# genjax-dev/genjax-chi

Measured on AMD Instinct MI355X. Metric: particles/sec, ImportanceK log-marginal-likelihood estimate (1e6 particles per GPU), higher is better.
Workload: dtype f32

## Files before the change

### genjax-chi_amd/csrc/gjx_device.hpp

```cpp
#pragma once
#ifndef __HIPCC_RTC__
#include <hip/hip_runtime.h>
#include <stdint.h>
#else
typedef unsigned char uint8_t;
typedef unsigned short uint16_t;
typedef int int32_t;
typedef unsigned int uint32_t;
typedef long long int64_t;
typedef unsigned long long uint64_t;
typedef unsigned long uintptr_t;
typedef unsigned long size_t;
#endif

#define GJX_DEV __device__ __forceinline__
#define GJX_HD __host__ __device__ __forceinline__

namespace gjx {

constexpr int kWave = 64;
constexpr int kBlock = 256;
#ifndef GJX_TILE
#define GJX_TILE 1024
#endif
// ... 237 lines not shown
  if (s.mode == 2) return s.parent;
  return split_at<IMPL>(s.parent, s.first + i);
}
template <int IMPL>
GJX_DEV void store_key(uint32_t* out, uint64_t i, Key k) {
  if (IMPL == 0) reinterpret_cast<uint2*>(out)[i] = make_uint2(k.k0, k.k1);
  else reinterpret_cast<uint4*>(out)[i] = make_uint4(k.k0, k.k1, k.l0, k.l1);
}

#if defined(__HIP_DEVICE_COMPILE__)
GJX_DEV float opq(float x) {
  asm volatile("" : "+v"(x));
  return x;
}
#else
GJX_HD float opq(float x) { return x; }
#endif

GJX_HD float m_log(float x) {
  uint32_t ix = f2u(x);
  int32_t e = 0;
  if (ix - 1u >= 0x7f7fffffu) {
    if ((ix << 1) == 0u) return -__builtin_inff();
    return ix == 0x7f800000u ? x : u2f(0x7fc00000u);
  }
  if (ix < 0x00800000u) {
    x = x * 8388608.0f;
    ix = f2u(x);
    e = -23;
  }
  const uint32_t t = ix - 0x3f3504f3u;
  e += (int32_t)t >> 23;
  const float m = u2f((t & 0x007fffffu) + 0x3f3504f3u);
  const float f = m - 1.0f;
  const float z = f * f;
  float p = 7.0376836292E-2f;
  p = __builtin_fmaf(p, f, -1.1514610310E-1f);
  p = __builtin_fmaf(p, f, 1.1676998740E-1f);
  p = __builtin_fmaf(p, f, -1.2420140846E-1f);
  p = __builtin_fmaf(p, f, 1.4249322787E-1f);
  p = __builtin_fmaf(p, f, -1.6668057665E-1f);
  p = __builtin_fmaf(p, f, 2.0000714765E-1f);
  p = __builtin_fmaf(p, f, -2.4999993993E-1f);
  p = __builtin_fmaf(p, f, 3.3333331174E-1f);
  float y = (p * f) * z;
  const float fe = (float)e;
  y = __builtin_fmaf(fe, -2.12194440e-4f, y);
  y = __builtin_fmaf(-0.5f, z, y);
  float r = f + y;
  r = __builtin_fmaf(fe, 0.693359375f, r);
  return r;
}

GJX_HD float m_log_normal(float x) {
  const uint32_t t = f2u(x) - 0x3f3504f3u;
  const int32_t e = (int32_t)t >> 23;
  const float m = u2f((t & 0x007fffffu) + 0x3f3504f3u);
  const float f = m - 1.0f;
  const float z = f * f;
  float p = 7.0376836292E-2f;
  p = __builtin_fmaf(p, f, -1.1514610310E-1f);
  p = __builtin_fmaf(p, f, 1.1676998740E-1f);
  p = __builtin_fmaf(p, f, -1.2420140846E-1f);
  p = __builtin_fmaf(p, f, 1.4249322787E-1f);
  p = __builtin_fmaf(p, f, -1.6668057665E-1f);
  p = __builtin_fmaf(p, f, 2.0000714765E-1f);
  p = __builtin_fmaf(p, f, -2.4999993993E-1f);
  p = __builtin_fmaf(p, f, 3.3333331174E-1f);
  float y = (p * f) * z;
  const float fe = (float)e;
  y = __builtin_fmaf(fe, -2.12194440e-4f, y);
  y = __builtin_fmaf(-0.5f, z, y);
  float r = f + y;
  r = __builtin_fmaf(fe, 0.693359375f, r);
  return r;
}

GJX_HD float m_exp_core(float x);
GJX_HD float m_exp(float x) {
  if (!(x >= -86.0f)) return 0.0f;
  if (x > 88.0f) x = 88.0f;
  return m_exp_core(x);
}
GJX_HD float m_exp_core(float x) {
  const float fx = __builtin_rintf(x * 1.44269504088896341f);
  x = __builtin_fmaf(fx, -0.693359375f, x);
  x = __builtin_fmaf(fx, 2.12194440e-4f, x);
  const float z = x * x;
  float p = 1.9875691500E-4f;
  p = __builtin_fmaf(p, x, 1.3981999507E-3f);
  p = __builtin_fmaf(p, x, 8.3334519073E-3f);
  p = __builtin_fmaf(p, x, 4.1665795894E-2f);
  p = __builtin_fmaf(p, x, 1.6666665459E-1f);
  p = __builtin_fmaf(p, x, 5.0000001201E-1f);
  const float y = __builtin_fmaf(p, z, x) + 1.0f;
  const int32_t n = (int32_t)fx;
  return u2f(f2u(y) + ((uint32_t)n << 23));
}

GJX_HD float e_exp(float x) {
  if (x != x) return x;
  if (x > 88.0f || x < -86.0f) {
    const float h = m_exp(x * 0.5f);
    return h * h;
  }
  return m_exp(x);
}

GJX_HD float e_max(float a, float b) { return (a != a) ? a : ((b != b) ? b : (a > b ? a : b)); }
GJX_HD float e_min(float a, float b) { return (a != a) ? a : ((b != b) ? b : (a < b ? a : b)); }

#if defined(GJX_FAST_MATH) && defined(__HIP_DEVICE_COMPILE__)
#define GJX_FAST_MATH_DEVICE 1
GJX_HD float d_exp(float x) { return __builtin_amdgcn_exp2f(x * 1.44269504088896341f); }
GJX_HD float d_exp_core(float x) { return d_exp(x); }
#else
GJX_HD float d_exp(float x) { return m_exp(x); }
GJX_HD float d_exp_core(float x) { return m_exp_core(x); }
#endif

GJX_HD float m_erfinv(float x) {
  float w = -m_log_normal((1.0f - x) * (1.0f + x));
  float p;
  if (w < 5.0f) {
    w = w - 2.5f;
    p = 2.81022636e-08f;
    p = __builtin_fmaf(p, w, 3.43273939e-07f);
    p = __builtin_fmaf(p, w, -3.5233877e-06f);
    p = __builtin_fmaf(p, w, -4.39150654e-06f);
    p = __builtin_fmaf(p, w, 0.00021858087f);
    p = __builtin_fmaf(p, w, -0.00125372503f);
    p = __builtin_fmaf(p, w, -0.00417768164f);
    p = __builtin_fmaf(p, w, 0.246640727f);
    p = __builtin_fmaf(p, w, 1.50140941f);
  } else {
    w = __builtin_sqrtf(w) - 3.0f;
    p = -0.000200214257f;
    p = __builtin_fmaf(p, w, 0.000100950558f);
    p = __builtin_fmaf(p, w, 0.00134934322f);
    p = __builtin_fmaf(p, w, -0.00367342844f);
    p = __builtin_fmaf(p, w, 0.00573950773f);
    p = __builtin_fmaf(p, w, -0.0076224613f);
    p = __builtin_fmaf(p, w, 0.00943887047f);
    p = __builtin_fmaf(p, w, 1.00167406f);
    p = __builtin_fmaf(p, w, 2.83297682f);
  }
  return p * x;
}

GJX_HD float m_lgamma(float x) {
  float p = 1.0f;
#pragma unroll
  for (int i = 0; i < 8; ++i) {
    if (x < 8.0f) {
      p = p * x;
      x = x + 1.0f;
    }
  }
  const float xi = 1.0f / x;
  const float xi2 = xi * xi;
  float s = __builtin_fmaf(xi2, 7.9365079365e-4f, -2.7777777778e-3f);
  s = __builtin_fmaf(s, xi2, 8.3333333333e-2f);
  s = s * xi;
  float r = (x - 0.5f) * m_log(x);
  r = r - x;
  r = r + 0.91893853320467f;
  r = r + s;
  r = r - m_log(p);
  return r;
}

GJX_HD float uniform01(uint32_t bits) { return u2f((bits >> 9) | 0x3F800000u) - 1.0f; }

GJX_HD float std_normal(uint32_t bits) {
  const float lo = -0.99999994f;
  float u = uniform01(bits) * 2.0f + lo;
  u = u > lo ? u : lo;
  return 1.41421356237309505f * m_erfinv(u);
}

struct BmEnt {
// ... 57 lines not shown
  {0xbf6b4b0cu, 0xbec9b953u}, {0xbf68bf3cu, 0xbed53641u}, {0xbf660f88u, 0xbee0924fu}, {0xbf633c5au, 0xbeebcbbbu}, \
  {0xbf604621u, 0xbef6e0cbu}, {0xbf5d2d53u, 0xbf00e7e4u}, {0xbf59f26au, 0xbf064b82u}, {0xbf5695e5u, 0xbf0b9a6bu}, \
  {0xbf531849u, 0xbf10d3cdu}, {0xbf4f7a1fu, 0xbf15f6d9u}, {0xbf4bbbf8u, 0xbf1b02c6u}, {0xbf47de65u, 0xbf1ff6cbu}, \
  {0xbf43e200u, 0xbf24d225u}, {0xbf3fc767u, 0xbf299415u}, {0xbf3b8f3bu, 0xbf2e3bdeu}, {0xbf373a23u, 0xbf32c8c9u}, \
  {0xbf32c8c9u, 0xbf373a23u}, {0xbf2e3bdeu, 0xbf3b8f3bu}, {0xbf299415u, 0xbf3fc767u}, {0xbf24d225u, 0xbf43e200u}, \
  {0xbf1ff6cbu, 0xbf47de65u}, {0xbf1b02c6u, 0xbf4bbbf8u}, {0xbf15f6d9u, 0xbf4f7a1fu}, {0xbf10d3cdu, 0xbf531849u}, \
  {0xbf0b9a6bu, 0xbf5695e5u}, {0xbf064b82u, 0xbf59f26au}, {0xbf00e7e4u, 0xbf5d2d53u}, {0xbef6e0cbu, 0xbf604621u}, \
  {0xbeebcbbbu, 0xbf633c5au}, {0xbee0924fu, 0xbf660f88u}, {0xbed53641u, 0xbf68bf3cu}, {0xbec9b953u, 0xbf6b4b0cu}, \
  {0xbebe1d4au, 0xbf6db293u}, {0xbeb263efu, 0xbf6ff573u}, {0xbea68f12u, 0xbf721352u}, {0xbe9aa086u, 0xbf740bddu}, \
  {0xbe8e9a22u, 0xbf75dec6u}, {0xbe827dc0u, 0xbf778bc5u}, {0xbe6c9a7fu, 0xbf791298u}, {0xbe541501u, 0xbf7a7302u}, \
  {0xbe3b6ecfu, 0xbf7baccdu}, {0xbe22abb6u, 0xbf7cbfc9u}, {0xbe09cf86u, 0xbf7dabccu}, {0xbde1bc2eu, 0xbf7e70b0u}, \
  {0xbdafb680u, 0xbf7f0e58u}, {0xbd7b2b74u, 0xbf7f84abu}, {0xbd16c32cu, 0xbf7fd397u}, {0xbc490e90u, 0xbf7ffb11u}, \
  {0x3c490e90u, 0xbf7ffb11u}, {0x3d16c32cu, 0xbf7fd397u}, {0x3d7b2b74u, 0xbf7f84abu}, {0x3dafb680u, 0xbf7f0e58u}, \
  {0x3de1bc2eu, 0xbf7e70b0u}, {0x3e09cf86u, 0xbf7dabccu}, {0x3e22abb6u, 0xbf7cbfc9u}, {0x3e3b6ecfu, 0xbf7baccdu}, \
  {0x3e541501u, 0xbf7a7302u}, {0x3e6c9a7fu, 0xbf791298u}, {0x3e827dc0u, 0xbf778bc5u}, {0x3e8e9a22u, 0xbf75dec6u}, \
  {0x3e9aa086u, 0xbf740bddu}, {0x3ea68f12u, 0xbf721352u}, {0x3eb263efu, 0xbf6ff573u}, {0x3ebe1d4au, 0xbf6db293u}, \
  {0x3ec9b953u, 0xbf6b4b0cu}, {0x3ed53641u, 0xbf68bf3cu}, {0x3ee0924fu, 0xbf660f88u}, {0x3eebcbbbu, 0xbf633c5au}, \
  {0x3ef6e0cbu, 0xbf604621u}, {0x3f00e7e4u, 0xbf5d2d53u}, {0x3f064b82u, 0xbf59f26au}, {0x3f0b9a6bu, 0xbf5695e5u}, \
  {0x3f10d3cdu, 0xbf531849u}, {0x3f15f6d9u, 0xbf4f7a1fu}, {0x3f1b02c6u, 0xbf4bbbf8u}, {0x3f1ff6cbu, 0xbf47de65u}, \
  {0x3f24d225u, 0xbf43e200u}, {0x3f299415u, 0xbf3fc767u}, {0x3f2e3bdeu, 0xbf3b8f3bu}, {0x3f32c8c9u, 0xbf373a23u}, \
  {0x3f373a23u, 0xbf32c8c9u}, {0x3f3b8f3bu, 0xbf2e3bdeu}, {0x3f3fc767u, 0xbf299415u}, {0x3f43e200u, 0xbf24d225u}, \
  {0x3f47de65u, 0xbf1ff6cbu}, {0x3f4bbbf8u, 0xbf1b02c6u}, {0x3f4f7a1fu, 0xbf15f6d9u}, {0x3f531849u, 0xbf10d3cdu}, \
  {0x3f5695e5u, 0xbf0b9a6bu}, {0x3f59f26au, 0xbf064b82u}, {0x3f5d2d53u, 0xbf00e7e4u}, {0x3f604621u, 0xbef6e0cbu}, \
  {0x3f633c5au, 0xbeebcbbbu}, {0x3f660f88u, 0xbee0924fu}, {0x3f68bf3cu, 0xbed53641u}, {0x3f6b4b0cu, 0xbec9b953u}, \
  {0x3f6db293u, 0xbebe1d4au}, {0x3f6ff573u, 0xbeb263efu}, {0x3f721352u, 0xbea68f12u}, {0x3f740bddu, 0xbe9aa086u}, \
  {0x3f75dec6u, 0xbe8e9a22u}, {0x3f778bc5u, 0xbe827dc0u}, {0x3f791298u, 0xbe6c9a7fu}, {0x3f7a7302u, 0xbe541501u}, \
  {0x3f7baccdu, 0xbe3b6ecfu}, {0x3f7cbfc9u, 0xbe22abb6u}, {0x3f7dabccu, 0xbe09cf86u}, {0x3f7e70b0u, 0xbde1bc2eu}, \
  {0x3f7f0e58u, 0xbdafb680u}, {0x3f7f84abu, 0xbd7b2b74u}, {0x3f7fd397u, 0xbd16c32cu}, {0x3f7ffb11u, 0xbc490e90u}, \
}
#if defined(__HIP_DEVICE_COMPILE__)
static __device__ const BmEnt g_bm_lg[64] = GJX_BM_LG_INIT;
static __device__ const BmEnt g_bm_cs[256] = GJX_BM_CS_INIT;
#else
static const BmEnt g_bm_lg[64] = GJX_BM_LG_INIT;
static const BmEnt g_bm_cs[256] = GJX_BM_CS_INIT;
#endif
#if defined(GJX_BM_LDS) && defined(__HIP_DEVICE_COMPILE__)
__shared__ BmEnt s_bm_lg[64];
__shared__ BmEnt s_bm_cs[256];
#ifndef GJX_BM_BLOCK
#error "GJX_BM_LDS needs GJX_BM_BLOCK: the size of the workgroups that call bm_stage()"
#endif
struct BmLoads {
  BmEnt c[256 / GJX_BM_BLOCK], l;
  GJX_DEV void bm_stage() const {
    constexpr int BD = GJX_BM_BLOCK, K = 256 / BD;
    const uint32_t t = threadIdx.x;
#pragma unroll
    for (int k = 0; k < K; ++k) s_bm_cs[t + (uint32_t)(k * BD)] = c[k];
    if (BD == 64 || t < 64u) s_bm_lg[t] = l;
    __syncthreads();
  }
};
GJX_DEV BmLoads bm_issue() {
  constexpr int BD = GJX_BM_BLOCK, K = 256 / BD;
  static_assert(BD == 64 || BD == 128 || BD == 256, "workgroups have 64, 128 or 256 threads");
  const uint32_t t = threadIdx.x;
  BmLoads r;
  r.l = BmEnt{0u, 0u};
#pragma unroll
  for (int k = 0; k < K; ++k) r.c[k] = g_bm_cs[t + (uint32_t)(k * BD)];
  if (BD == 64 || t < 64u) r.l = g_bm_lg[t];
  return r;
}
GJX_DEV void bm_stage() { bm_issue().bm_stage(); }
#define GJX_BM_LG s_bm_lg
#define GJX_BM_CS s_bm_cs
#else
#define GJX_BM_LG g_bm_lg
#define GJX_BM_CS g_bm_cs
#endif
GJX_HD float sqrt_pos(float x) {
#if defined(__HIP_DEVICE_COMPILE__) && !defined(GJX_GENERAL_SQRT)
  const float y = __builtin_amdgcn_rsqf(__builtin_fmaxf(x, 1e-30f));
  float s = x * y, h = 0.5f * y;
  const float e = __builtin_fmaf(-h, s, 0.5f);
  h = __builtin_fmaf(h, e, h);
  s = __builtin_fmaf(s, e, s);
  return __builtin_fmaf(__builtin_fmaf(-s, s, x), h, s);
#else
  return __builtin_sqrtf(x);
#endif
}
GJX_HD void bm_pair(uint32_t w_radius, uint32_t w_angle, float& z_cos, float& z_sin) {
  const float uw = (float)w_radius + 1.0f;
#ifdef GJX_FAST_MATH_DEVICE
  {
    const float u = uw * 2.3283064365386963e-10f;
    const float rf = __builtin_amdgcn_sqrtf(-1.38629436111989062f * __builtin_amdgcn_logf(u));
    const float tf = (float)(w_angle >> 8) * 5.9604644775390625e-08f;
    z_cos = rf * __builtin_amdgcn_cosf(tf);
    z_sin = rf * __builtin_amdgcn_sinf(tf);
    return;
  }
#endif
  const uint32_t t = f2u(uw) - (0x3f3504f3u + (32u << 23));
  const BmEnt lg = GJX_BM_LG[(t >> 17) & 63u];
  const float m = u2f((t & 0x007fffffu) + 0x3f3504f3u);
  const float fe = (float)((int32_t)t >> 23);
  const float q = __builtin_fmaf(m, u2f(lg.a), -1.0f);
  float p = __builtin_fmaf(q, -0.25f, 0.333333343f);
  p = __builtin_fmaf(p, q, -0.5f);
  const float l1 = __builtin_fmaf(p, q * q, q);
  const float lu = __builtin_fmaf(fe, 0.693147182f, u2f(lg.b)) + l1;
  const float r = sqrt_pos(-2.0f * lu);
  const BmEnt cs = GJX_BM_CS[w_angle >> 24];
  const float d = __builtin_fmaf((float)((w_angle >> 8) & 0xffffu), 3.74507035e-07f, -0.0122718466f);
  const float d2 = d * d;
  const float sd = __builtin_fmaf(d2 * d, -0.166666672f, d);
  const float cd = __builtin_fmaf(d2, __builtin_fmaf(d2, 0.0416666679f, -0.5f), 1.0f);
  const float ca = u2f(cs.a), sa = u2f(cs.b);
  z_cos = r * __builtin_fmaf(ca, cd, -(sa * sd));
  z_sin = r * __builtin_fmaf(sa, cd, ca * sd);
}
constexpr uint32_t kTagTwin = 0x54u;
template <int IMPL>
GJX_HD float site_normal(const Stream<IMPL>& st) {
  if (IMPL == 0 || !st.hf) return std_normal(st.bits32(0));
  float zc, zs;
  uint32_t o[4];
  if ((st.k.l0 | st.k.l1) == 0u) {
    philox4x32(st.k.k0, st.k.k1, 0u, 0u, st.f >> 2, kTagTwin, o[0], o[1], o[2], o[3]);
    const uint32_t sel = st.f & 3u;
    bm_pair(philox_single_draw(st.k, st.f), sel == 0 ? o[0] : (sel == 1 ? o[1] : (sel == 2 ? o[2] : o[3])), zc, zs);
    return zc;
  }
  philox_pair_block(st.k, st.f >> 1, o);
  if (st.f & 1u) bm_pair(o[2], o[3], zc, zs);
  else bm_pair(o[0], o[1], zc, zs);
  return ((st.k.l0 - 1u) & 1u) ? zs : zc;
}

template <int IMPL>
GJX_HD void smc_quad_normals(Key step_key, uint64_t g, float (&z)[4]) {
  uint32_t w[4];
  smc_quad_bits<IMPL>(step_key, g, w);
  if (IMPL == 0) {
#pragma unroll
    for (int u = 0; u < 4; ++u) z[u] = std_normal(w[u]);
  } else {
    bm_pair(w[0], w[1], z[0], z[1]);
    bm_pair(w[2], w[3], z[2], z[3]);
  }
}
template <int IMPL>
GJX_HD float smc_slot_normal(Key step_key, uint64_t j) {
  if (IMPL == 0) return std_normal(smc_slot_bits<IMPL>(step_key, j));
  float z[4];
  smc_quad_normals<IMPL>(step_key, j >> 2, z);
  const uint32_t sel = (uint32_t)j & 3u;
  return sel == 0 ? z[0] : (sel == 1 ? z[1] : (sel == 2 ? z[2] : z[3]));
}

GJX_HD float normal_rs(float scale) { return 1.0f / scale; }
GJX_HD float normal_lognorm(float scale) { return 0.91893853320467f + m_log(scale); }
GJX_HD float logpdf_normal_pre(float x, float loc, float rs, float lognorm) {
  const float d = x * rs - loc * rs;
  return (-0.5f * d) * d - lognorm;
}
GJX_HD float logpdf_normal(float x, float loc, float scale) {
  return logpdf_normal_pre(x, loc, normal_rs(scale), normal_lognorm(scale));
}
GJX_HD float normal_resid_pow2(float x, float loc, float rs) { return __builtin_fmaf(-rs, loc, x * rs); }
GJX_HD float normal_halfsq(float d, float lognorm) { return __builtin_fmaf(d * d, -0.5f, -lognorm); }
struct NormalExactCuts {};
GJX_HD float logpdf_normal_pre(float x, float loc, float rs, float lognorm, NormalExactCuts) {
  return normal_halfsq(normal_resid_pow2(x, loc, rs), lognorm);
}
GJX_HD float xlogy(float a, float y) { return a == 0.0f ? 0.0f : a * m_log(y); }
GJX_HD float gamma_lognorm(float conc, float rate) { return m_lgamma(conc) - conc * m_log(rate); }
GJX_HD float logpdf_gamma_pre(float x, float conc, float rate, float lognorm) {
  return (xlogy(conc - 1.0f, x) - rate * x) - lognorm;
}
GJX_HD float logpdf_gamma(float x, float conc, float rate) {
  return logpdf_gamma_pre(x, conc, rate, gamma_lognorm(conc, rate));
}
GJX_HD float beta_lbeta(float a, float b) { return (m_lgamma(a) + m_lgamma(b)) - m_lgamma(a + b); }
GJX_HD float logpdf_beta_pre(float x, float a, float b, float lbeta) {
  return (xlogy(a - 1.0f, x) + xlogy(b - 1.0f, 1.0f - x)) - lbeta;
}
GJX_HD float logpdf_beta(float x, float a, float b) {
  return logpdf_beta_pre(x, a, b, beta_lbeta(a, b));
}
GJX_HD float logpdf_bernoulli(bool e, float p) { return e ? m_log(p) : m_log(1.0f - p); }

template <int IMPL>
GJX_DEV float gamma_dv(const Stream<IMPL>& st, int which, float conc) {
  const bool boost = conc < 1.0f;
  const float a = boost ? conc + 1.0f : conc;
  const float d = a - 0.33333334f;
  const float c = 1.0f / __builtin_sqrtf(9.0f * d);
  float v = 1.0f;
  for (int att = 0; att < 64; ++att) {
    uint32_t w0, w1;
    st.words((uint32_t)(1 + 2 * att + which), w0, w1);
    const float x = std_normal(w0);
// ... 59 lines not shown
  v = (t * t) * t;
  const float u = uniform01(w1);
  float rhs = (0.5f * x) * x + d;
  rhs = rhs - d * v;
  rhs = rhs + d * m_log(v);
  return m_log(u) < rhs;
}
template <int IMPL, int P>
GJX_DEV void std_gamma_multi(const Stream<IMPL> (&st)[P], int which, const float (&conc)[P], float (&out)[P]) {
  float d[P], c[P], v[P];
  int att[P];
  bool done[P];
#pragma unroll
  for (int u = 0; u < P; ++u) {
    const float a = conc[u] < 1.0f ? conc[u] + 1.0f : conc[u];
    d[u] = a - 0.33333334f;
    c[u] = 1.0f / __builtin_sqrtf(9.0f * d[u]);
    v[u] = 1.0f;
  }
#pragma unroll
  for (int u = 0; u < P; ++u) {
    done[u] = gamma_attempt<IMPL>(st[u], which, 0, d[u], c[u], v[u]);
    att[u] = 1;
  }
  for (;;) {
    int pick = -1;
#pragma unroll
    for (int u = P - 1; u >= 0; --u) pick = (!done[u] && att[u] < 64) ? u : pick;
#if defined(__HIP_DEVICE_COMPILE__)
    if (__ballot(pick >= 0) == 0) break;
#else
    if (pick < 0) break;
#endif
    if (pick >= 0) {
      Stream<IMPL> s = st[0];
      float dd = d[0], cc = c[0], vv = v[0];
      int aa = att[0];
#pragma unroll
      for (int u = 1; u < P; ++u)
        if (pick == u) { s = st[u]; dd = d[u]; cc = c[u]; vv = v[u]; aa = att[u]; }
      const bool ok = gamma_attempt<IMPL>(s, which, aa, dd, cc, vv);
#pragma unroll
      for (int u = 0; u < P; ++u)
        if (pick == u) { v[u] = vv; att[u] = aa + 1; done[u] = ok; }
    }
  }
#pragma unroll
  for (int u = 0; u < P; ++u) {
    float g = d[u] * v[u];
    if (conc[u] < 1.0f) {
      uint32_t w0, w1;
      st[u].words(0u, w0, w1);
      const float ub = uniform01(which ? w1 : w0);
      g = g * m_exp(m_log(ub) / conc[u]);
    }
    out[u] = g;
  }
}

GJX_HD uint64_t fixw(float lw, float m, int frac) {
  if (lw == m) return (uint64_t)1 << frac;
  const float d = lw - m;
  if (!(d >= -80.0f)) return 0;
  const float s = m_exp(d);
  const float t = s * u2f((uint32_t)(127 + frac) << 23);
  return (uint64_t)__builtin_rintf(t);
}
constexpr int kRowFrac = 30;
constexpr int32_t kRowEmpty = -(1 << 30);
constexpr int kLseBuckets = 64;
constexpr int kLseRecordWords = 1 + kLseBuckets;
GJX_HD int32_t row_anchor(float m) {
  if (!(m > -__builtin_inff())) return kRowEmpty;
  float t = m * 1.44269504088896341f;
  t = t > 16777216.0f ? 16777216.0f : (t < -16777216.0f ? -16777216.0f : t);
  return (int32_t)__builtin_ceilf(t);
}
GJX_HD uint64_t rowfix(float lw, int32_t e) {
#if defined(__HIP_DEVICE_COMPILE__)
  {
    const float fe = (float)e;
    float d = __builtin_fmaf(-fe, 0.693359375f, lw);
    d = __builtin_fmaf(-fe, -2.12194440e-4f, d);
    d = d > 1.0f ? 1.0f : d;
    const bool live = e != kRowEmpty && lw > -__builtin_inff() && d >= -86.0f;
    const uint32_t q = (uint32_t)__builtin_rintf(d_exp_core(live ? d : 0.0f) * 1073741824.0f);
    return live ? q : 0u;
  }
#endif
  if (e == kRowEmpty || !(lw > -__builtin_inff())) return 0;
  const float fe = (float)e;
  float d = __builtin_fmaf(-fe, 0.693359375f, lw);
  d = __builtin_fmaf(-fe, -2.12194440e-4f, d);
  d = d > 1.0f ? 1.0f : d;
  return (uint64_t)(uint32_t)__builtin_rintf(d_exp(d) * 1073741824.0f);
}

GJX_HD uint32_t cat_fix(float l, float m) {
  if (l == m) return 1u << kCatFrac;
  const float d = l - m;
  if (!(d >= -80.0f)) return 0u;
  return (uint32_t)__builtin_rintf(m_exp(d) * 8388608.0f);
}
GJX_HD int frac_bits(uint64_t n_total) {
  int lg = 0;
  while (lg < 63 && ((uint64_t)1 << lg) < n_total) ++lg;
  const int f = 62 - lg;
  return f > 40 ? 40 : (f < 8 ? 8 : f);
}
GJX_HD float gumbel_from_bits(uint32_t bits) {
  const float tiny = 1.17549435e-38f;
  float u = uniform01(bits) + tiny;
  u = u > tiny ? u : tiny;
  return -m_log(-m_log(u));
}

#if defined(__HIP_DEVICE_COMPILE__)
GJX_DEV float jrow_max(const float* l, uint32_t K) {
  float m = l[0];
  for (uint32_t c = 1; c < K; ++c) m = l[c] > m ? l[c] : m;
  return m;
}
GJX_DEV float jrow_lse(const float* l, uint32_t K) {
  const float m = jrow_max(l, K);
  float acc = 0.0f;
  for (uint32_t c = 0; c < K; ++c) acc = acc + m_exp(l[c] - m);
  return m + m_log(acc);
}
GJX_DEV int32_t jcat_invcdf(const float* l, uint32_t K, uint32_t bits) {
  const float m = jrow_max(l, K);
  uint64_t Q = 0;
  for (uint32_t c = 0; c < K; ++c) Q += cat_fix(l[c], m);
  const uint64_t thr = (uint64_t)bits * (Q >> 32) + (((uint64_t)bits * (Q & 0xffffffffu)) >> 32);
  uint64_t C = 0;
  for (uint32_t c = 0; c < K; ++c) {
    C += cat_fix(l[c], m);
    if (C > thr) return (int32_t)c;
  }
  return (int32_t)(K - 1);
}
typedef unsigned jv4u_t __attribute__((ext_vector_type(4)));
GJX_DEV uint4 jguide_load(const uint4* p) {
  const uint64_t a = (uint64_t)(uintptr_t)p;
  const uint64_t first = ((uint64_t)(uint32_t)__builtin_amdgcn_readfirstlane((int)(uint32_t)(a >> 32)) << 32) |
                         (uint64_t)(uint32_t)__builtin_amdgcn_readfirstlane((int)(uint32_t)a);
  const uint64_t base = first - (1ull << 30);
  __amdgpu_buffer_rsrc_t rs = __builtin_amdgcn_make_buffer_rsrc((void*)(uintptr_t)base, 0, 0x7fffffff, 0x00020000);
  const jv4u_t v = __builtin_amdgcn_raw_buffer_load_b128(rs, (int)(uint32_t)(a - base), 0, 0);
  return make_uint4(v[0], v[1], v[2], v[3]);
}
GJX_DEV int32_t jcat_invcdf_gb(const uint4* guide, const uint2* ent, uint32_t K, uint32_t bits, int sh, uint32_t& lpb) {
  const uint4 g = jguide_load(guide + (bits >> sh));
  const uint32_t c0 = g.y & 511u, c1 = (g.y >> 9) & 511u;
  if (bits <= g.x) {
    lpb = g.z;
    return (int32_t)c0;
  }
  if (!(g.y >> 18)) {
    lpb = g.w;
    return (int32_t)c1;
  }
  const uint64_t thr = ((uint64_t)bits * (uint64_t)ent[K - 1].x) >> 32;
  uint32_t c = c1;
  uint2 e = ent[c];
  while (c < K - 1 && (uint64_t)e.x <= thr) {
    ++c;
    e = ent[c];
  }
  lpb = e.y;
  return (int32_t)c;
}
template <int IMPL>
GJX_DEV int32_t jcat_gumbel(const float* l, uint32_t K, const Stream<IMPL>& st) {
  int32_t best = 0;
  float bv = -__builtin_inff();
  for (uint32_t c = 0; c < K; ++c) {
    const float v = l[c] + gumbel_from_bits(st.bits32(c));
    if (v > bv || c == 0) {
      bv = v;
      best = (int32_t)c;
    }
  }
  return best;
}
#endif

GJX_HD int64_t teeth_below(uint64_t C, double scale, double u0, int64_t n_out) {
  const double P = (double)C * scale;
  const double c = __builtin_ceil(P - u0);
  if (!(c > 0.0)) return 0;
  if (c >= (double)n_out) return n_out;
  return (int64_t)(int32_t)c;
}
GJX_HD double u0_from_bits(uint64_t U) { return (double)(U >> 11) * 0x1.0p-53; }

template <int CTRL, int ROW_MASK, int BANK_MASK>
GJX_DEV uint32_t dpp_u32(uint32_t identity, uint32_t v) {
  return (uint32_t)__builtin_amdgcn_update_dpp((int)identity, (int)v, CTRL, ROW_MASK, BANK_MASK, false);
}
template <int CTRL, int ROW_MASK, int BANK_MASK>
GJX_DEV uint64_t dpp_u64(uint64_t identity, uint64_t v) {
  const uint32_t lo = dpp_u32<CTRL, ROW_MASK, BANK_MASK>((uint32_t)identity, (uint32_t)v);
  const uint32_t hi = dpp_u32<CTRL, ROW_MASK, BANK_MASK>((uint32_t)(identity >> 32), (uint32_t)(v >> 32));
  return ((uint64_t)hi << 32) | lo;
}
constexpr int kDppRowShr1 = 0x111, kDppRowShr2 = 0x112, kDppRowShr3 = 0x113, kDppRowShr4 = 0x114, kDppRowShr8 = 0x118,
              kDppRowBcast15 = 0x142, kDppRowBcast31 = 0x143, kDppWaveShr1 = 0x138;
#define GJX_WAVE_SCAN_BODY(T, MOV)                                               \
  T r = op(v, MOV<kDppRowShr1, 0xf, 0xf>(id, v));                                \
  r = op(r, MOV<kDppRowShr2, 0xf, 0xf>(id, v));                                  \
  r = op(r, MOV<kDppRowShr3, 0xf, 0xf>(id, v));                                  \
  r = op(r, MOV<kDppRowShr4, 0xf, 0xe>(id, r));                                  \
  r = op(r, MOV<kDppRowShr8, 0xf, 0xc>(id, r));                                  \
  r = op(r, MOV<kDppRowBcast15, 0xa, 0xf>(id, r));                               \
  r = op(r, MOV<kDppRowBcast31, 0xc, 0xf>(id, r));                               \
  return r;
template <class Op>
GJX_DEV uint32_t wave_scan_u32(uint32_t v, uint32_t id, Op op) { GJX_WAVE_SCAN_BODY(uint32_t, dpp_u32) }
template <class Op>
GJX_DEV uint64_t wave_scan_u64(uint64_t v, uint64_t id, Op op) { GJX_WAVE_SCAN_BODY(uint64_t, dpp_u64) }
#undef GJX_WAVE_SCAN_BODY
GJX_DEV uint32_t wave_last_u32(uint32_t v) { return (uint32_t)__builtin_amdgcn_readlane((int)v, 63); }
GJX_DEV uint64_t wave_last_u64(uint64_t v) {
  return ((uint64_t)wave_last_u32((uint32_t)(v >> 32)) << 32) | wave_last_u32((uint32_t)v);
}
GJX_DEV float wave_max(float v) {
  v = v == v ? v : -__builtin_inff();
  const uint32_t r = wave_scan_u32(f2u(v), f2u(-__builtin_inff()),
                                   [](uint32_t a, uint32_t b) { return u2f(b) > u2f(a) ? b : a; });
  return u2f(wave_last_u32(r));
}
GJX_DEV uint64_t wave_sum(uint64_t v) {
  return wave_last_u64(wave_scan_u64(v, 0, [](uint64_t a, uint64_t b) { return a + b; }));
}
GJX_DEV int wave_sum_int(int v) {
  return (int)wave_last_u32(wave_scan_u32((uint32_t)v, 0u, [](uint32_t a, uint32_t b) { return a + b; }));
}
GJX_DEV float block_max(float v, float* sh) {
  v = wave_max(v);
  const int w = threadIdx.x >> 6;
  __syncthreads();
  if ((threadIdx.x & 63) == 0) sh[w] = v;
  __syncthreads();
  float r = sh[0];
#pragma unroll
  for (int i = 1; i < kBlock / kWave; ++i) r = sh[i] > r ? sh[i] : r;
  return r;
}
GJX_DEV uint64_t block_sum(uint64_t v, uint64_t* sh) {
  v = wave_sum(v);
  const int w = threadIdx.x >> 6;
  __syncthreads();
  if ((threadIdx.x & 63) == 0) sh[w] = v;
  __syncthreads();
  uint64_t r = 0;
#pragma unroll
  for (int i = 0; i < kBlock / kWave; ++i) r += sh[i];
  return r;
}
GJX_DEV uint64_t wave_scan_incl(uint64_t v) {
  return wave_scan_u64(v, 0, [](uint64_t a, uint64_t b) { return a + b; });
}
GJX_DEV uint64_t wave_scan_incl_52(uint64_t v) {
  const uint32_t lo = wave_scan_u32((uint32_t)v & 0x3ffffffu, 0u, [](uint32_t a, uint32_t b) { return a + b; });
  const uint32_t hi = wave_scan_u32((uint32_t)(v >> 26), 0u, [](uint32_t a, uint32_t b) { return a + b; });
  return ((uint64_t)hi << 26) + lo;
}
GJX_DEV uint64_t wave_sum_52(uint64_t v) { return wave_last_u64(wave_scan_incl_52(v)); }
GJX_DEV uint64_t block_scan_excl(uint64_t v, uint64_t* sh, uint64_t& total) {
  const uint64_t incl = wave_scan_incl(v);
  const int w = threadIdx.x >> 6, lane = threadIdx.x & 63;
  __syncthreads();
  if (lane == 63) sh[w] = incl;
  __syncthreads();
  uint64_t base = 0, tot = 0;
#pragma unroll
  for (int i = 0; i < kBlock / kWave; ++i) {
    if (i < w) base += sh[i];
    tot += sh[i];
  }
  total = tot;
  return base + incl - v;
}

GJX_DEV int block_scan_max_excl(int v, int* sh) {
  const int lane = threadIdx.x & 63, w = threadIdx.x >> 6;
  const int incl = (int)wave_scan_u32((uint32_t)v, 0u, [](uint32_t a, uint32_t b) { return b > a ? b : a; });
  int excl = (int)dpp_u32<kDppWaveShr1, 0xf, 0xf>(0u, (uint32_t)incl);
  __syncthreads();
  if (lane == 63) sh[w] = incl;
  __syncthreads();
#pragma unroll
  for (int i = 0; i < kBlock / kWave; ++i)
    if (i < w) excl = sh[i] > excl ? sh[i] : excl;
  return excl;
}
GJX_DEV int block_sum_int(int v, int* sh) {
  v = wave_sum_int(v);
  __syncthreads();
  if ((threadIdx.x & 63) == 0) sh[threadIdx.x >> 6] = v;
  __syncthreads();
  int r = 0;
#pragma unroll
  for (int i = 0; i < kBlock / kWave; ++i) r += sh[i];
  return r;
}

constexpr int kMaxFilters = 16;
struct FilterBatch {
  uint32_t n_filters = 0;
  uint32_t tiles = 0;
  uint64_t stride = 0;
  uint64_t mq_stride = 0;
// ... 1421 lines not shown
```

### genjax-chi_amd/csrc/gjx_hip.hip

```cpp
#include "../../include/gjx.h"
#include "../../include/gjx_guided.h"
#include "../../include/gjx_backsim.h"
#include "../../include/gjx_backmove.h"
#include "../../include/gjx_smc_params.h"
#include "../../include/gjx_csmc.h"
#include "../../include/gjx_temper.h"
#include "../../include/gjx_plate.h"
#include "../../include/gjx_pointwise.h"
#include "../../include/gjx_temper_cov.h"
#define GJX_PHILOX_PLAIN_XOR 1
#include "gjx_device.hpp"

#include <hip/hip_runtime.h>
#include <math.h>
#include <new>
#include <string.h>

#include "gjx_plan_jit.hpp"

using namespace gjx;

namespace {

inline int launch_status() { return hipGetLastError() == hipSuccess ? GJX_OK : GJX_ERR_LAUNCH; }
// ... 1581 lines not shown
    scaled[c] = p * (uint64_t)K;
    alias[c] = (uint16_t)c;
    q += p;
  }
  q = wave_sum(q);
  if ((tid & 63) == 0) sh_q[tid >> 6] = q;
  __syncthreads();
  const uint64_t Q = sh_q[0] + sh_q[1];
  if (tid == 0) {
    uint32_t hs = 0, ts = 0, hl = 0, tl = 0;
    for (int c = 0; c < K; ++c) {
      if (scaled[c] < Q) small[ts++] = (uint16_t)c;
      else large[tl++] = (uint16_t)c;
    }
    while (hs < ts && hl < tl) {
      const uint32_t sc = small[hs++], g = large[hl];
      alias[sc] = (uint16_t)g;
      scaled[g] -= Q - scaled[sc];
      if (scaled[g] < Q) {
        ++hl;
        small[ts++] = (uint16_t)g;
      }
    }
  } else if (tid == 64) {
    const float* o = obs_logits + (size_t)r * K;
    sh_lse = row_lse(o, (uint32_t)K);
  }
  __syncthreads();
  uint32_t* row = trans_alias + (size_t)r * K;
  for (int c = tid; c < K; c += 128) {
    const uint32_t thr = alias[c] == c ? 0xffffffu : (uint32_t)((scaled[c] << 24) / Q);
    row[c] = (thr << 8) | alias[c];
    obs_logp[(size_t)r * K + c] = obs_logits[(size_t)r * K + c] - sh_lse;
  }
}

struct Carver {
  char* p;
  size_t left;
  bool ok = true;
  template <class T>
  T* take(size_t count) {
    const size_t bytes = (count * sizeof(T) + 255) & ~(size_t)255;
    if (!ok || bytes > left) {
      ok = false;
      return nullptr;
    }
    T* r = reinterpret_cast<T*>(p);
    p += bytes;
    left -= bytes;
    return r;
  }
};
inline size_t pad256(size_t b) { return (b + 255) & ~(size_t)255; }

template <int OP>
__global__ __launch_bounds__(kBlock) void k_map_f32(const float* x, float c, float* out, uint64_t n) {
  const uint64_t i0 = ((uint64_t)blockIdx.x * kBlock + threadIdx.x) * 4;
#pragma unroll
  for (int r = 0; r < 4; ++r) {
    const uint64_t i = i0 + r;
    if (i < n) {
      const float v = x[i];
      out[i] = OP == GJX_MAP_EXP ? e_exp(v) : OP == GJX_MAP_LOG ? m_log(v) : OP == GJX_MAP_DIV ? v / c : OP == GJX_MAP_RDIV ? c / v
               : OP == GJX_MAP_SQRT ? __builtin_sqrtf(v) : __builtin_fabsf(v);
    }
  }
}

__global__ __launch_bounds__(kBlock) void k_sqrt_pos_sweep(uint32_t lo, uint64_t count, unsigned long long* out) {
  unsigned long long bad = 0, first = ~0ull;
  for (uint64_t i = (uint64_t)blockIdx.x * kBlock + threadIdx.x; i < count; i += (uint64_t)gridDim.x * kBlock) {
    const uint32_t b = lo + (uint32_t)i;
    if (f2u(sqrt_pos(u2f(b))) != f2u(__builtin_sqrtf(u2f(b)))) {
      ++bad;
      first = first < b ? first : b;
    }
  }
  if (bad) {
    atomicAdd(&out[0], bad);
    atomicMin(&out[1], first);
  }
}
}

static int copy_source_out(const std::string& src, char* buf, size_t buf_len, size_t* needed) {
  if (needed) *needed = src.size() + 1;
  if (buf && buf_len > 0) {
    const size_t k = src.size() < buf_len - 1 ? src.size() : buf_len - 1;
    memcpy(buf, src.data(), k);
    buf[k] = 0;
  }
  return GJX_OK;
}
static int version_out(int* major, int* minor, int maj, int min) {
  if (major) *major = maj;
  if (minor) *minor = min;
  return GJX_OK;
}
extern "C" {

int gjx_version(int* major, int* minor) { return version_out(major, minor, GJX_VERSION_MAJOR, GJX_VERSION_MINOR); }
const char* gjx_backend_name(void) { return "hip-gfx950"; }
int gjx_frac_bits(uint64_t n_total) { return frac_bits(n_total); }
uint64_t gjx_smc_tile(void) { return kTile; }
uint64_t gjx_num_tiles(uint64_t n) { return ntiles_of(n); }
uint64_t gjx_num_max_partials(uint64_t n) { return nrows_of(n); }

size_t gjx_workspace_bytes(int op, uint64_t n) {
  const uint64_t nt = ntiles_of(n);
  switch (op) {
    case GJX_OP_LOGSUMEXP: return pad256(nrows_of(n) * 4) + pad256(nt * 8) + 1024;
    case GJX_OP_CATEGORICAL_INDEX:
    case GJX_OP_RESAMPLE:
      return pad256(nt * 4) + 2 * pad256(nt * 8) + pad256(n * 8) + pad256(nt * 160) + pad256(prefix_words(nt) * 8) + 2048;
    case GJX_OP_SMC:
      return (GJX_SMC_MAX_STATE + 3) * pad256(n * 4) + 2 * (pad256(nt * 16) + pad256(nt * 128) + pad256(nt * 16)) + 2 * pad256(prefix_words(nt) * 8) + 4096 +
             pad256(256 * (256 + 64) * 4) + pad256(256 * 256 * 4) + 1024;
    default: return 0;
  }
}

#define GJX_DISPATCH_IMPL(impl, KERNEL, ...)  \
  do {                                        \
    if ((impl) == 0) KERNEL<0> __VA_ARGS__;   \
    else KERNEL<1> __VA_ARGS__;               \
  } while (0)

int gjx_rng_keys(const gjx_keys* k, uint64_t n, uint32_t* out, gjx_stream s) {
  if (!keys_ok(k) || (!out && n)) return GJX_ERR_INVALID;
  if (n == 0) return GJX_OK;
  GJX_DISPATCH_IMPL(k->impl, k_rng_keys, <<<grid_for(n), kBlock, 0, S(s)>>>(key_src(k), n, out));
  return launch_status();
}
int gjx_rng_split_each(const gjx_keys* k, uint64_t n, uint32_t m, uint32_t* out, gjx_stream s) {
  if (!keys_ok(k) || (!out && n) || m == 0) return GJX_ERR_INVALID;
  if (n == 0) return GJX_OK;
  GJX_DISPATCH_IMPL(k->impl, k_rng_split_each, <<<grid_for(n * m), kBlock, 0, S(s)>>>(key_src(k), n, m, out));
  return launch_status();
}
int gjx_rng_bits(const gjx_keys* k, uint32_t sub, uint64_t n, uint32_t* out, gjx_stream s) {
  if (!keys_ok(k) || (!out && n)) return GJX_ERR_INVALID;
  if (n == 0) return GJX_OK;
  GJX_DISPATCH_IMPL(k->impl, k_rng_bits, <<<grid_for(n), kBlock, 0, S(s)>>>(key_src(k), sub, n, out));
  return launch_status();
}

int gjx_sample_logpdf_normal(const gjx_keys* k, gjx_f32 loc, gjx_f32 scale, float* value_out,
                             float* score_out, uint64_t n, gjx_stream s) {
  if (!keys_ok(k) || !value_out) return GJX_ERR_INVALID;
  if (n == 0) return GJX_OK;
  GJX_DISPATCH_IMPL(k->impl, k_sample_normal,
                    <<<grid_for(n), kBlock, 0, S(s)>>>(key_src(k), opnd(loc), opnd(scale), value_out, score_out, n));
  return launch_status();
}
int gjx_sample_logpdf_gamma(const gjx_keys* k, gjx_f32 concentration, gjx_f32 rate,
                            float* value_out, float* score_out, uint64_t n, gjx_stream s) {
  if (!keys_ok(k) || !value_out) return GJX_ERR_INVALID;
  if (n == 0) return GJX_OK;
  GJX_DISPATCH_IMPL(k->impl, k_sample_gamma,
                    <<<grid_for(n), kBlock, 0, S(s)>>>(key_src(k), opnd(concentration), opnd(rate), value_out, score_out, n));
  return launch_status();
}
int gjx_sample_logpdf_beta(const gjx_keys* k, gjx_f32 a, gjx_f32 b, float* value_out,
                           float* score_out, uint64_t n, gjx_stream s) {
  if (!keys_ok(k) || !value_out) return GJX_ERR_INVALID;
// ... 84 lines not shown
    for (uint32_t k = c + 1; k < K; ++k)
      if (row[k].x > row[c].x) { cn = k; break; }
    const uint32_t last_bits = (uint32_t)((((uint64_t)g + 1) << sh) - 1);
    const uint64_t thr_last = ((uint64_t)last_bits * (uint64_t)C) >> 32;
    const bool multi = cn != c && (uint64_t)row[cn].x <= thr_last;
    const uint32_t bm1 = C == 0 ? 0xffffffffu : (uint32_t)(((((uint64_t)row[c].x) << 32) - 1) / (uint64_t)C);
    guide4[((size_t)r << gbits) + g] = make_uint4(row[c].x == 0 ? 0xffffffffu : bm1, c | (cn << 9) | ((multi ? 1u : 0u) << 18), row[c].y, row[cn].y);
  }
}
static void cat_tables_prepare(CSite* sites, int n, std::vector<void*>* owned) {
  bool any = false;
  for (int q = 0; q < n; ++q) {
    CSite& st = sites[q];
    if (st.dist != GJX_DIST_CATEGORICAL || st.cat_ent || st.cat_logp_t || !st.logits || st.n_cat > 511 || st.n_rows < 1) continue;
    const size_t rows = (size_t)st.n_rows;
    const unsigned grid = ((unsigned)rows + 63) / 64;
    if (!gjx_jit::sampled_mode(st.observed) && st.obs.kind != GJX_ARG_INPUT) {
      float* lt = nullptr;
      if (hipMalloc(&lt, sizeof(float) * rows * (size_t)st.n_cat) != hipSuccess) { (void)hipGetLastError(); continue; }
      k_cat_prepare<<<grid, 64>>>(st.logits, (uint32_t)rows, (uint32_t)st.n_cat, nullptr, nullptr, lt, 0);
      owned->push_back(lt);
      st.cat_logp_t = lt;
      any = true;
      continue;
    }
    uint2* ent = nullptr;
    uint4* guide4 = nullptr;
    int gbits = 8;
    while ((1 << gbits) < 4 * st.n_cat && gbits < 11) ++gbits;
    while (gbits > 8 && (sizeof(uint4) << gbits) * rows > ((size_t)2 << 20)) --gbits;
    if (hipMalloc(&ent, sizeof(uint2) * rows * (size_t)st.n_cat) != hipSuccess || hipMalloc(&guide4, (sizeof(uint4) << gbits) * rows) != hipSuccess) {
      (void)hipGetLastError();
      if (ent) (void)hipFree(ent);
      continue;
    }
    k_cat_prepare<<<grid, 64>>>(st.logits, (uint32_t)rows, (uint32_t)st.n_cat, ent, guide4, nullptr, gbits);
    owned->push_back(ent);
    owned->push_back(guide4);
    st.cat_ent = ent;
    st.cat_guide4 = guide4;
    st.cat_gbits = gbits;
    any = true;
  }
  if (any && hipDeviceSynchronize() != hipSuccess) (void)hipGetLastError();
}
static void free_owned(std::vector<void*>& owned) {
  for (void* p : owned) (void)hipFree(p);
  owned.clear();
}
struct SiteTable {
  CSite* sites;
  int n;
};
extern "C++" template <class Build>
static bool compiled_once(std::mutex& mu, gjx_jit::Module& c, std::initializer_list<SiteTable> tables, std::vector<void*>* owned,
                          Build build) {
  if (c.state == 0) {
    std::lock_guard<std::mutex> lock(mu);
    if (c.state == 0) {
      for (const SiteTable& t : tables) cat_tables_prepare(t.sites, t.n, owned);
      c.state = build() ? 1 : -1;
    }
  }
  return c.state == 1;
}

struct ExprStore {
  gjx_expr_op ops[GJX_MAX_SITES][2][GJX_MAX_EXPR_OPS];
};

struct gjx_plan {
  int n_sites;
  int n_slots;
  int dist_mask;
  uint32_t flags;
  int n_params;
  int max_param;
  PlanParams prm;
  CSite host[GJX_MAX_SITES];
  CSite* dev;
  gjx_jit::Compiled jit[4];
  gjx_jit::Compiled jit_tail[4];
  gjx_jit::Compiled jit_wt[2];
  std::vector<void*> dev_owned;
  std::mutex jit_mu;
  ExprStore expr;
  bool has_expr;
  int expr_max_input;
  gjx_jit::ScopeInfo scopes;
};

static bool expr_ok(const gjx_arg& a, int s, int n_state, int n_obs, bool allow_state, bool allow_param = false) {
  const gjx_expr_op* ops = reinterpret_cast<const gjx_expr_op*>(a.table);
  if (!ops || a.ref < 1 || a.ref > GJX_MAX_EXPR_OPS) return false;
  int depth = 0;
  for (int k = 0; k < a.ref; ++k) {
    const int r = ops[k].ref;
    switch (ops[k].op) {
      case GJX_EXPR_CONST: ++depth; break;
      case GJX_EXPR_SITE: if (r < 0 || r >= s) return false; ++depth; break;
      case GJX_EXPR_INPUT: if (n_state >= 0 || r < 0 || r >= 16) return false; ++depth; break;
      case GJX_EXPR_PARAM: if ((n_state >= 0 && !allow_param) || r < 0 || r >= GJX_MAX_PARAMS) return false; ++depth; break;
      case GJX_EXPR_STATE: if (n_state < 0 || !allow_state || r < 0 || r >= n_state) return false; ++depth; break;
      case GJX_EXPR_OBS: if (n_state < 0 || r < 0 || r >= n_obs) return false; ++depth; break;
      case GJX_EXPR_ADD: case GJX_EXPR_SUB: case GJX_EXPR_MUL: case GJX_EXPR_DIV: case GJX_EXPR_MAX: case GJX_EXPR_MIN:
      case GJX_EXPR_LT: case GJX_EXPR_LE: case GJX_EXPR_EQ:
        if (depth < 2) return false;
        --depth;
        break;
      case GJX_EXPR_SELECT:
        if (depth < 3) return false;
        depth -= 2;
        break;
      case GJX_EXPR_NEG: case GJX_EXPR_EXP: case GJX_EXPR_LOG: case GJX_EXPR_SQRT: case GJX_EXPR_ABS: if (depth < 1) return false; break;
      default: return false;
    }
    if (depth > 8) return false;
  }
  return depth == 1;
}

static bool arg_ok(const gjx_arg& a, int s, int n_state = -1, int n_obs = -1, bool allow_state = false, bool allow_param = false) {
  switch (a.kind) {
    case GJX_ARG_EXPR: return expr_ok(a, s, n_state, n_obs, allow_state, allow_param);
    case GJX_ARG_CONST: return true;
    case GJX_ARG_SITE: return a.ref >= 0 && a.ref < s;
    case GJX_ARG_INPUT: return n_state < 0 && a.ref >= 0 && a.ref < 16;
    case GJX_ARG_TABLE: return a.ref >= 0 && a.ref < s && a.table != nullptr;
    case GJX_ARG_STATE: return allow_state && a.ref >= 0 && a.ref < n_state;
    case GJX_ARG_OBS: return n_obs >= 0 && a.ref >= 0 && a.ref < n_obs;
    case GJX_ARG_PARAM: return (n_state < 0 || allow_param) && a.ref >= 0 && a.ref < GJX_MAX_PARAMS;
    default: return false;
  }
}
static CArg carg(const gjx_arg& a) { return CArg{a.kind, a.ref, 0, a.ref, a.scale, a.offset, a.table}; }

static bool convert_site(const gjx_site& st, int s, CSite& c, int n_state = -1, int n_obs = -1,
                         bool allow_state = false, bool allow_guided = false, bool allow_next = false, bool allow_param = false) {
  if (st.observed > (allow_guided ? GJX_SITE_GUIDED : 1)) return false;
  bool ok = st.dist >= 0 && st.dist <= GJX_DIST_CATEGORICAL && arg_ok(st.arg[0], s, n_state, n_obs, allow_state, allow_param);
  const bool two_args = st.dist != GJX_DIST_BERNOULLI && st.dist != GJX_DIST_CATEGORICAL;
  if (ok && two_args) ok = arg_ok(st.arg[1], s, n_state, n_obs, allow_state, allow_param);
  if (ok && st.observed == GJX_SITE_GUIDED) {
    ok = st.obs.kind == GJX_ARG_SITE && st.obs.ref >= 0 && st.obs.ref < s && st.obs.scale == 1.0f && st.obs.offset == 0.0f;
  } else if (ok && st.observed && st.observed != GJX_SITE_PROPOSED) {
    if (n_state < 0) ok = st.obs.kind == GJX_ARG_CONST || (st.obs.kind == GJX_ARG_INPUT && st.obs.ref >= 0 && st.obs.ref < 16) ||
                          (st.obs.kind == GJX_ARG_PARAM && st.obs.ref >= 0 && st.obs.ref < GJX_MAX_PARAMS);
    else ok = st.obs.kind == GJX_ARG_CONST || (st.obs.kind == GJX_ARG_OBS && st.obs.ref >= 0 && st.obs.ref < n_obs) ||
              (allow_param && st.obs.kind == GJX_ARG_PARAM && st.obs.ref >= 0 && st.obs.ref < GJX_MAX_PARAMS) ||
              (allow_next && st.obs.kind == GJX_ARG_NEXT && st.obs.ref >= 0 && st.obs.ref < n_state && st.obs.scale == 1.0f &&
               st.obs.offset == 0.0f);
  }
  if (ok && st.dist == GJX_DIST_CATEGORICAL)
    ok = st.logits && st.n_cat > 0 && st.n_rows > 0 && (st.cat_mode == 0 || st.cat_mode == 1) && st.arg[0].kind != GJX_ARG_EXPR;
  if (!ok) return false;
  memset(&c, 0, sizeof(c));
  c.dist = st.dist; c.observed = st.observed; c.out_col = st.out_col;
  c.n_cat = st.n_cat; c.n_rows = st.n_rows; c.cat_mode = st.cat_mode;
  c.slot = -1;
  c.a0 = carg(st.arg[0]); c.a1 = carg(st.arg[1]); c.obs = carg(st.obs);
  if (!two_args) c.a1.kind = GJX_ARG_CONST;
  c.logits = st.logits;
  const bool c0 = st.arg[0].kind == GJX_ARG_CONST, c1 = st.arg[1].kind == GJX_ARG_CONST;
  const bool u0 = c0 || st.arg[0].kind == GJX_ARG_PARAM, u1 = c1 || st.arg[1].kind == GJX_ARG_PARAM;
  if (st.dist == GJX_DIST_NORMAL && c1) {
    c.pre = 1; c.pre0 = normal_rs(st.arg[1].offset); c.pre1 = normal_lognorm(st.arg[1].offset);
// ... 81 lines not shown
        a->ref_is_int = p->host[a->ref].dist >= GJX_DIST_BERNOULLI;
        a->ref = site_slot[a->ref];
      }
    if (last_use[s] < 0) continue;
    int slot = -1;
    for (int k = 0; k < n_slots; ++k)
      if (slot_free_at[k] <= s) { slot = k; break; }
    if (slot < 0) slot = n_slots++;
    slot_free_at[slot] = last_use[s] + 1;
    site_slot[s] = slot;
    c.slot = slot;
  }
  p->n_slots = n_slots;
  p->has_expr = expr_adopt(p->host, n_sites, &p->expr);
  p->expr_max_input = expr_max_ref(p->host, n_sites, GJX_EXPR_INPUT);
  const int mp = expr_max_ref(p->host, n_sites, GJX_EXPR_PARAM);
  if (mp > p->max_param) p->max_param = mp;
  *out = p;
  return GJX_OK;
}

int gjx_plan_create_scoped(const gjx_site* sites, int n_sites, const gjx_scope* scopes, int n_scopes, uint32_t flags,
                           gjx_plan** out) {
  gjx_plan* p = nullptr;
  const int rc = gjx_plan_create_ex(sites, n_sites, flags, &p);
  if (rc) return rc;
  if (!gjx_jit::derive_scopes(sites, n_sites, scopes, n_scopes, p->scopes)) {
    gjx_plan_destroy(p);
    return GJX_ERR_INVALID;
  }
  *out = p;
  return GJX_OK;
}

static void plan_derive_params(PlanParams& prm, const CSite* sites, int n_sites) {
  auto val = [&](const CArg& a) {
    if (a.kind == GJX_ARG_CONST) return a.offset;
    const float t = a.scale * prm.p[a.ref];
    return t + a.offset;
  };
  for (int q = 0; q < n_sites; ++q) {
    const CSite& c = sites[q];
    if (c.pre != 2) continue;
    if (c.dist == GJX_DIST_NORMAL) {
      prm.d[2 * q] = normal_rs(val(c.a1));
      prm.d[2 * q + 1] = normal_lognorm(val(c.a1));
    } else if (c.dist == GJX_DIST_GAMMA) {
      prm.d[2 * q + 1] = gamma_lognorm(val(c.a0), val(c.a1));
    } else {
      prm.d[2 * q + 1] = beta_lbeta(val(c.a0), val(c.a1));
    }
  }
}
int gjx_plan_set_params(gjx_plan* p, const float* params, int n_params) {
  if (!p || n_params < 0 || n_params > GJX_MAX_PARAMS || (n_params && !params) || n_params <= p->max_param) return GJX_ERR_INVALID;
  for (int k = 0; k < n_params; ++k) p->prm.p[k] = params[k];
  p->n_params = n_params;
  plan_derive_params(p->prm, p->host, p->n_sites);
  return GJX_OK;
}

static int plan_device_table(gjx_plan* p) {
  std::lock_guard<std::mutex> lock(p->jit_mu);
  if (p->dev) return GJX_OK;
  if (hipMalloc(&p->dev, sizeof(CSite) * (size_t)p->n_sites) != hipSuccess) {
    p->dev = nullptr;
    return GJX_ERR_NO_DEVICE;
  }
  if (hipMemcpy(p->dev, p->host, sizeof(CSite) * (size_t)p->n_sites, hipMemcpyHostToDevice) != hipSuccess) {
    (void)hipFree(p->dev);
    p->dev = nullptr;
    return GJX_ERR_LAUNCH;
  }
  return GJX_OK;
}

static int jit_form_pref() {
  const char* e = std::getenv("GJX_JIT_FORM");
  if (e && !strcmp(e, "one")) return 1;
  if (e && !strcmp(e, "pair")) return 2;
  return 4;
}
static int jit_waves_hint(int P) { return P == 2 ? 6 : 0; }
static void plan_gen_setup(gjx_jit::Gen<CSite, CArg>& g, const gjx_plan* p, int impl, int form, bool fused_tail, bool wt_stores, int min_waves) {
  g.impl = impl; g.sites = p->host; g.n_sites = p->n_sites; g.laned = form >= 2; g.pairs_per_lane = form == 4 ? 2 : 1;
  g.sc = p->scopes.n_scopes > 0 ? &p->scopes : nullptr;
  g.fast_math = (p->flags & GJX_PLAN_FAST_MATH) != 0;
  g.fused_tail = fused_tail;
  g.wt_stores = wt_stores;
  g.min_waves = min_waves;
}
int gjx_plan_specialized_source(const gjx_plan* p, int impl, char* buf, size_t buf_len, size_t* needed) {
  const bool fused_tail = (impl & GJX_SOURCE_FUSED_TAIL) != 0, wt_stores = (impl & GJX_SOURCE_WT_STORES) != 0;
  impl &= ~(GJX_SOURCE_FUSED_TAIL | GJX_SOURCE_WT_STORES);
  if (!p || (impl != 0 && impl != 1)) return GJX_ERR_INVALID;
  const int form = impl == 1 ? jit_form_pref() : 1;
  gjx_jit::Gen<CSite, CArg> g;
  plan_gen_setup(g, p, impl, form, fused_tail, wt_stores, jit_waves_hint(form));
  gjx_jit::TableScope ts;
  return copy_source_out(g.run(), buf, buf_len, needed);
}

int gjx_plan_compile_check(const gjx_plan* p, int impl) {
  const bool fused_tail = (impl & GJX_SOURCE_FUSED_TAIL) != 0, wt_stores = (impl & GJX_SOURCE_WT_STORES) != 0;
  impl &= ~(GJX_SOURCE_FUSED_TAIL | GJX_SOURCE_WT_STORES);
  if (!p || (impl != 0 && impl != 1)) return GJX_ERR_INVALID;
  for (int form = 1; form <= (impl == 1 ? 4 : 1); form *= 2) {
    gjx_jit::Gen<CSite, CArg> g;
    plan_gen_setup(g, p, impl, form, fused_tail, wt_stores && form == 4, jit_waves_hint(form));
    gjx_jit::TableScope ts;
    if (!gjx_jit::compile_only(g.run(), gjx_jit::PlanKind::importance)) return GJX_ERR_UNSUPPORTED;
  }
  return GJX_OK;
}
int gjx_plan_destroy(gjx_plan* p) {
  if (!p) return GJX_OK;
  if (p->dev) (void)hipFree(p->dev);
  for (auto& c : p->jit) c.release();
  for (auto& c : p->jit_tail) c.release();
  for (auto& c : p->jit_wt) c.release();
  free_owned(p->dev_owned);
  delete p;
  return GJX_OK;
}

static gjx_jit::Compiled& plan_compiled(gjx_plan* mp, const gjx_keys* pk, int lane_particles, bool fused_tail = false, bool one_pass = false) {
  const bool pairable = pk->impl == 1 && pk->mode == 1 && pk->parent_lane == 0 && (pk->first & 1) == 0;
  int P = pairable ? (lane_particles < jit_form_pref() ? lane_particles : jit_form_pref()) : 1;
  if (P == 3) P = 2;
  const bool laned = P >= 2;
  const bool wt_stores = one_pass && P == 4;
  gjx_jit::Compiled& c = wt_stores ? mp->jit_wt[fused_tail ? 1 : 0] : (fused_tail ? mp->jit_tail : mp->jit)[P == 4 ? 3 : (laned ? 2 : pk->impl)];
  compiled_once(mp->jit_mu, c, {{mp->host, mp->n_sites}}, &mp->dev_owned, [&] {
    auto build = [&](int min_waves) {
      gjx_jit::Gen<CSite, CArg> g;
      plan_gen_setup(g, mp, pk->impl, P, fused_tail, wt_stores, min_waves);
      gjx_jit::TableScope ts;
      const std::string src = g.run();
      c.block = g.block;
      c.rows_per_block = g.rows_per_block;
      c.tabs = ts.reg.tables();
      return c.load(src, gjx_jit::PlanKind::importance, {g.kname()}, {&c.fn});
    };
    const int hint = laned ? jit_waves_hint(P) : 0;
    bool ok = build(hint);
    if (ok && std::getenv("GJX_PLAN_JIT_VERBOSE")) {
      int regs = 0;
      if (hipFuncGetAttribute(&regs, HIP_FUNC_ATTRIBUTE_NUM_REGS, c.fn) != hipSuccess) (void)hipGetLastError();
      fprintf(stderr, "gjx jit: %d particle(s) per lane%s%s: %d registers per lane\n", P, fused_tail ? ", fused tail" : "", wt_stores ? ", write-through stores" : "", regs);
    }
    if (ok && hint > 0) {
      int scratch = 0;
      const hipError_t qe = hipFuncGetAttribute(&scratch, HIP_FUNC_ATTRIBUTE_LOCAL_SIZE_BYTES, c.fn);
      if (qe != hipSuccess) (void)hipGetLastError();
      if (std::getenv("GJX_PLAN_JIT_VERBOSE")) fprintf(stderr, "gjx jit: waves-per-SIMD hint %d: query %d, scratch %d B\n", hint, (int)qe, scratch);
      if (qe != hipSuccess || scratch > 32) {
        ok = build(0);
      }
    }
    if (!ok) {
      (void)hipGetLastError();
      fprintf(stderr, "[gjx] plan specialisation FAILED (hiprtc compile or module load; impl %d, %d particle(s) per lane). "
                      "gjx_importance_run returns GJX_ERR_JIT; set GJX_PLAN_JIT_VERBOSE=1 for the compiler log, GJX_PLAN_JIT=0 "
                      "or GJX_PLAN_JIT_FALLBACK=1 to run the (7x slower) table interpreter instead.\n", pk->impl, P);
    }
    return ok;
  });
  return c;
}
static bool jit_fallback_allowed() {
  static const bool allow = [] {
    const char* e = std::getenv("GJX_PLAN_JIT_FALLBACK");
    return e && e[0] == '1';
  }();
  return allow;
}
int gjx_plan_prepare(gjx_plan* p, const gjx_keys* pk) {
  if (!p || !keys_ok(pk)) return GJX_ERR_INVALID;
  if (!gjx_jit::enabled()) return p->has_expr ? GJX_ERR_UNSUPPORTED : plan_device_table(p);
  bool ok = plan_compiled(p, pk, 1).state == 1;
  ok = plan_compiled(p, pk, 2).state == 1 && ok;
  ok = plan_compiled(p, pk, 4).state == 1 && ok;
  ok = plan_compiled(p, pk, 4, false, true).state == 1 && ok;
  if (ok) return GJX_OK;
  return jit_fallback_allowed() && !p->has_expr ? plan_device_table(p) : GJX_ERR_JIT;
}

int gjx_map_f32(int op, const float* x, float c, float* out, uint64_t n, gjx_stream s) {
  if (!x || !out || op < GJX_MAP_EXP || op > GJX_MAP_ABS) return GJX_ERR_INVALID;
  if (n == 0) return GJX_OK;
  const unsigned grid = (unsigned)((n + 4ull * kBlock - 1) / (4ull * kBlock));
  switch (op) {
    case GJX_MAP_EXP: k_map_f32<GJX_MAP_EXP><<<grid, kBlock, 0, S(s)>>>(x, c, out, n); break;
    case GJX_MAP_LOG: k_map_f32<GJX_MAP_LOG><<<grid, kBlock, 0, S(s)>>>(x, c, out, n); break;
    case GJX_MAP_DIV: k_map_f32<GJX_MAP_DIV><<<grid, kBlock, 0, S(s)>>>(x, c, out, n); break;
    case GJX_MAP_SQRT: k_map_f32<GJX_MAP_SQRT><<<grid, kBlock, 0, S(s)>>>(x, c, out, n); break;
    case GJX_MAP_ABS: k_map_f32<GJX_MAP_ABS><<<grid, kBlock, 0, S(s)>>>(x, c, out, n); break;
    default: k_map_f32<GJX_MAP_RDIV><<<grid, kBlock, 0, S(s)>>>(x, c, out, n); break;
  }
  return launch_status();
}

static int importance_launch(const gjx_plan* p, const gjx_keys* pk, int32_t n_pass, uint64_t pass_stride,
                             uint64_t row_stride, const float* const* input_cols, int n_input_cols,
                             void* const* value_cols, int n_value_cols, float* score, float* logw, uint64_t n,
                             float* max_partials, int32_t* row_e, uint64_t* row_s, const gjx_lse_out* lse,
                             gjx_stream s) {
  if (!p || !pk || (!logw && !row_e) || n_input_cols < 0 || n_input_cols > 16 || n_value_cols < 0 ||
      n_value_cols > GJX_MAX_SITES || ((row_e == nullptr) != (row_s == nullptr)) || (lse && (!row_e || !lse->tickets)))
    return GJX_ERR_INVALID;
  for (int32_t b = 0; b < n_pass; ++b)
    if (!keys_ok(pk + b) || pk[b].has_fold) return GJX_ERR_INVALID;
  RunCols cols;
  memset(&cols, 0, sizeof(cols));
  for (int c = 0; c < n_input_cols; ++c) cols.in[c] = input_cols[c];
  for (int c = 0; c < n_value_cols; ++c) cols.out[c] = value_cols[c];
  for (int q = 0; q < p->n_sites; ++q) {
    const CSite& st = p->host[q];
    if (st.out_col >= n_value_cols) return GJX_ERR_INVALID;
    if (st.out_col >= 0 && !cols.out[st.out_col]) return GJX_ERR_INVALID;
    if (st.a0.kind == GJX_ARG_INPUT && st.a0.ref >= n_input_cols) return GJX_ERR_INVALID;
    if (st.a1.kind == GJX_ARG_INPUT && st.a1.ref >= n_input_cols) return GJX_ERR_INVALID;
    if (st.observed && st.obs.kind == GJX_ARG_INPUT && st.obs.ref >= n_input_cols) return GJX_ERR_INVALID;
  }
  if (p->max_param >= p->n_params) return GJX_ERR_INVALID;
  if (p->expr_max_input >= n_input_cols) return GJX_ERR_INVALID;
  if (n == 0) return GJX_OK;
  KeySrc k = key_src(pk);
  if (gjx_jit::enabled()) {
    uintptr_t al = (uintptr_t)logw | (uintptr_t)score | (uintptr_t)(4 * pass_stride) | (uintptr_t)(4 * n);
    for (int c = 0; c < n_value_cols; ++c) al |= (uintptr_t)value_cols[c];
    const int lane_particles = (al & 15) == 0 ? 4 : ((al & 7) == 0 ? 2 : 1);
    gjx_jit::Compiled& c = plan_compiled(const_cast<gjx_plan*>(p), pk, lane_particles, lse != nullptr, n_pass <= 1);
    if (c.state != 1 && (!jit_fallback_allowed() || p->has_expr || p->scopes.n_scopes > 0)) return GJX_ERR_JIT;
    if (c.state == 1) {
      uint64_t nn = n;
      LseTail tail{nullptr, nullptr, nullptr, nullptr, nullptr, nullptr, 0.0f};
      if (lse) tail = LseTail{lse->e, lse->q, lse->lse, lse->record, lse->tickets, lse->lse_shifted, lse->shift};
      PassBatch bt;
      memset(&bt, 0, sizeof bt);
      bt.n_pass = (uint32_t)n_pass;
      bt.rows_per_pass = (uint32_t)nrows_of(n);
      bt.pass_stride = pass_stride;
      bt.row_stride = row_stride;
      for (int32_t b = 0; b < n_pass; ++b) { bt.parent[b][0] = pk[b].parent[0]; bt.parent[b][1] = pk[b].parent[1]; }
      PlanParams prm = p->prm;
      PlanTables tabs = c.tabs;
      void* args[] = {&k, &cols, &score, &logw, &nn, &max_partials, &row_e, &row_s, &tail, &bt, &prm, &tabs};
      const uint64_t rows = (nrows_of(n) + c.rows_per_block - 1) / c.rows_per_block;
      return launch_generated(c.fn, rows > 0x7fffffffull ? 0x7fffffffull : rows, (unsigned)n_pass, (unsigned)c.block, s, args);
    }
  }
  if (p->has_expr || p->scopes.n_scopes > 0) return GJX_ERR_UNSUPPORTED;
  {
    const int rc = plan_device_table(const_cast<gjx_plan*>(p));
    if (rc) return rc;
  }
  const size_t lds = sizeof(uint32_t) * (size_t)(p->n_slots > 0 ? p->n_slots : 1) * kImpTile;
  const int m = p->dist_mask;
  for (int32_t b = 0; b < n_pass; ++b) {
    KeySrc kb = key_src(pk + b);
    RunCols cb = cols;
    for (int c = 0; c < n_value_cols; ++c)
      if (cb.out[c]) cb.out[c] = (char*)cb.out[c] + 4 * (size_t)b * pass_stride;
    float* sc_b = score ? score + (size_t)b * pass_stride : nullptr;
    float* lw_b = logw + (size_t)b * pass_stride;
    float* mp_b = max_partials ? max_partials + (size_t)b * row_stride : nullptr;
    int32_t* re_b = row_e ? row_e + (size_t)b * row_stride : nullptr;
    uint64_t* rs_b = row_s ? row_s + (size_t)b * row_stride : nullptr;
#define GJX_LAUNCH_IMPORTANCE(IMPL, MASK) \
  k_importance<IMPL, MASK><<<(unsigned)((n + kImpTile - 1) / kImpTile), kBlock, lds, S(s)>>>(p->dev, p->n_sites, kb, cb, sc_b, lw_b, n, mp_b, re_b, rs_b, p->prm)
    if (pk->impl == 0) {
      if ((m & ~kMaskNormal) == 0) GJX_LAUNCH_IMPORTANCE(0, kMaskNormal);
      else if ((m & ~kMaskReal) == 0) GJX_LAUNCH_IMPORTANCE(0, kMaskReal);
      else GJX_LAUNCH_IMPORTANCE(0, kMaskAll);
    } else {
      if ((m & ~kMaskNormal) == 0) GJX_LAUNCH_IMPORTANCE(1, kMaskNormal);
      else if ((m & ~kMaskReal) == 0) GJX_LAUNCH_IMPORTANCE(1, kMaskReal);
      else GJX_LAUNCH_IMPORTANCE(1, kMaskAll);
    }
#undef GJX_LAUNCH_IMPORTANCE
  }
  if (lse) k_lse_rows<<<1, kBlock, 0, S(s)>>>(row_e, row_s, nrows_of(n), 0, lse->e, lse->q, lse->lse, lse->record);
  return launch_status();
}

int gjx_importance_run(const gjx_plan* p, const gjx_keys* pk, const float* const* input_cols,
                       int n_input_cols, void* const* value_cols, int n_value_cols, float* score,
                       float* logw, uint64_t n, float* max_partials, int32_t* row_e, uint64_t* row_s,
                       const gjx_lse_out* lse, gjx_stream s) {
  return importance_launch(p, pk, 1, 0, 0, input_cols, n_input_cols, value_cols, n_value_cols, score, logw, n,
                           max_partials, row_e, row_s, lse, s);
}

int gjx_importance_estimate(const gjx_estimate_io* io, uint32_t k0, uint32_t k1, uint64_t lane, float* out, float shift,
                            gjx_stream s) {
  if (!io || !io->plan || !io->row_e || !io->row_s || !io->lse.tickets || !out || (io->impl != 0 && io->impl != 1) ||
      (io->impl == 0 && lane != 0))
    return GJX_ERR_INVALID;
  for (int q = 0; q < io->plan->n_sites; ++q)
    if (io->plan->host[q].out_col >= 0) return GJX_ERR_INVALID;
  Key k{k0, k1, (uint32_t)lane, (uint32_t)(lane >> 32)};
  k = io->impl == 0 ? split_at<0>(split_at<0>(k, 1), 1) : split_at<1>(split_at<1>(k, 1), 1);
  gjx_keys pk;
  memset(&pk, 0, sizeof pk);
  pk.impl = io->impl;
  pk.mode = 1;
  pk.parent[0] = k.k0; pk.parent[1] = k.k1;
  pk.parent_lane = ((uint64_t)k.l1 << 32) | k.l0;
  gjx_lse_out lse = io->lse;
  lse.lse_shifted = out;
  lse.shift = shift;
  return importance_launch(io->plan, &pk, 1, 0, 0, io->input_cols, io->n_input_cols, nullptr, 0, nullptr, nullptr, io->n, nullptr,
                           io->row_e, io->row_s, &lse, s);
}

// ... 894 lines not shown
      for (int q = 0; q < n; ++q) {
        const CSite& c = sites[q];
        if (c.pre != 2) continue;
        if (c.dist == GJX_DIST_NORMAL) {
          d[2 * q] = normal_rs(val(c.a1));
          d[2 * q + 1] = normal_lognorm(val(c.a1));
        } else if (c.dist == GJX_DIST_GAMMA) {
          d[2 * q + 1] = gamma_lognorm(val(c.a0), val(c.a1));
        } else {
          d[2 * q + 1] = beta_lbeta(val(c.a0), val(c.a1));
        }
      }
    };
    derive(p->init, p->n_init, row + P);
    derive(p->step, p->n_step, row + P + 2 * p->n_init);
  }
  p->n_rows = n_rows;
  p->rows_dirty = true;
  return GJX_OK;
}
static void smc_plan_free_rows(gjx_smc_plan* p) {
  for (int i = 0; i < gjx_smc_plan::kStage; ++i) {
    if (p->stage_ev[i]) (void)hipEventDestroy(p->stage_ev[i]);
    if (p->stage[i]) (void)hipHostFree(p->stage[i]);
    p->stage_ev[i] = nullptr;
    p->stage[i] = nullptr;
  }
  if (p->dev_rows) (void)hipFree(p->dev_rows);
  p->dev_rows = nullptr;
}
static int smc_plan_upload_rows(gjx_smc_plan* p, int F, gjx_stream s) {
  std::lock_guard<std::mutex> lock(p->mu);
  if (p->n_rows < 1 || (p->n_rows != 1 && p->n_rows != F) || F > kMaxFilters) return GJX_ERR_INVALID;
  const size_t L = (size_t)p->row_len();
  const size_t table_bytes = sizeof(float) * L * (size_t)kMaxFilters;
  if (!p->dev_rows) {
    bool ok = hipMalloc((void**)&p->dev_rows, table_bytes) == hipSuccess;
    for (int i = 0; ok && i < gjx_smc_plan::kStage; ++i)
      ok = hipHostMalloc((void**)&p->stage[i], table_bytes, hipHostMallocDefault) == hipSuccess &&
           hipEventCreateWithFlags(&p->stage_ev[i], hipEventDisableTiming) == hipSuccess;
    if (!ok) {
      (void)hipGetLastError();
      smc_plan_free_rows(p);
      return GJX_ERR_LAUNCH;
    }
  }
  const int slot = p->stage_next;
  p->stage_next = (slot + 1) % gjx_smc_plan::kStage;
  if (hipEventSynchronize(p->stage_ev[slot]) != hipSuccess) {
    (void)hipGetLastError();
    return GJX_ERR_LAUNCH;
  }
  for (int f = 0; f < F; ++f)
    memcpy(p->stage[slot] + (size_t)f * L, p->rows.data() + (p->n_rows == 1 ? 0 : (size_t)f * L), sizeof(float) * L);
  if (hipMemcpyAsync(p->dev_rows, p->stage[slot], sizeof(float) * L * (size_t)F, hipMemcpyHostToDevice, S(s)) != hipSuccess ||
      hipEventRecord(p->stage_ev[slot], S(s)) != hipSuccess) {
    (void)hipGetLastError();
    return GJX_ERR_LAUNCH;
  }
  p->rows_dirty = false;
  return GJX_OK;
}
int gjx_smc_plan_destroy(gjx_smc_plan* p) {
  if (!p) return GJX_OK;
  smc_plan_free_rows(p);
  for (auto& c : p->jit) c.release();
  for (auto& c : p->jit_peers) c.release();
  for (auto& c : p->jit_cond) c.release();
  free_owned(p->dev_owned);
  if (p->dev_init) (void)hipFree(p->dev_init);
  if (p->dev_step) (void)hipFree(p->dev_step);
  delete p;
  return GJX_OK;
}
int gjx_jit_compile_source(const char* source) {
  if (!source) return GJX_ERR_INVALID;
  return gjx_jit::compile_only(source, gjx_jit::PlanKind::smc ) ? GJX_OK : GJX_ERR_JIT;
}
int gjx_debug_sqrt_pos_sweep(uint32_t lo_bits, uint32_t hi_bits, uint64_t* out, gjx_stream s) {
  if (!out || hi_bits < lo_bits) return GJX_ERR_INVALID;
  const uint64_t count = (uint64_t)hi_bits - lo_bits + 1;
  const uint64_t blocks = (count + kBlock - 1) / kBlock;
  k_sqrt_pos_sweep<<<(unsigned)(blocks < 2048 ? blocks : 2048), kBlock, 0, S(s)>>>(lo_bits, count, reinterpret_cast<unsigned long long*>(out));
  return launch_status();
}
int gjx_jit_stats(uint64_t* compiles, uint64_t* cached_modules, uint64_t* evictions) {
  gjx_jit::ModuleCache& mc = gjx_jit::ModuleCache::get();
  std::lock_guard<std::mutex> lock(mc.mu);
  if (compiles) *compiles = mc.compiles;
  if (cached_modules) *cached_modules = mc.map.size();
  if (evictions) *evictions = mc.evictions;
  return GJX_OK;
}

int gjx_jit_routes(uint64_t* child_compiles, uint64_t* inproc_compiles, uint64_t* child_failures, uint64_t* spawn_failures) {
  gjx_jit::RouteCounters& r = gjx_jit::routes();
  if (child_compiles) *child_compiles = r.child.load();
  if (inproc_compiles) *inproc_compiles = r.inproc.load();
  if (child_failures) *child_failures = r.child_failures.load();
  if (spawn_failures) *spawn_failures = r.spawn_failures.load();
  return GJX_OK;
}

static std::string smc_plan_source(const gjx_smc_plan* plan, int impl, PlanTables* tabs = nullptr, bool peers = false, bool cond = false) {
  gjx_jit::GenSmc<CSite, CArg> g;
  g.peers = peers;
  if (cond) {
    g.cond = true;
    (void)g.csmc_components(plan->init, plan->n_init, plan->init_state, plan->n_state, g.ret_init);
    (void)g.csmc_components(plan->step, plan->n_step, plan->next_state, plan->n_state, g.ret_step);
  }
  g.impl = impl; g.init_sites = plan->init; g.n_init = plan->n_init; g.step_sites = plan->step;
  g.n_step = plan->n_step; g.init_state = plan->init_state; g.next_state = plan->next_state; g.n_state = plan->n_state;
  g.sc_init = plan->init_scopes.n_scopes > 0 ? &plan->init_scopes : nullptr;
  g.sc_step = plan->step_scopes.n_scopes > 0 ? &plan->step_scopes : nullptr;
  g.n_params = plan->n_params;
  return gjx_jit::generated_source(g, tabs);
}
int gjx_smc_plan_source(const gjx_smc_plan* p, int impl, char* buf, size_t buf_len, size_t* needed) {
  if (!p || (impl != 0 && impl != 1)) return GJX_ERR_INVALID;
  return copy_source_out(smc_plan_source(p, impl), buf, buf_len, needed);
}
int gjx_smc_plan_compile_check(const gjx_smc_plan* p, int impl) {
  if (!p || (impl != 0 && impl != 1)) return GJX_ERR_INVALID;
  if (std::getenv("GJX_PLAN_JIT_DUMP")) fprintf(stderr, "%s\n", smc_plan_source(p, impl).c_str());
  return gjx_jit::compile_only(smc_plan_source(p, impl), gjx_jit::PlanKind::smc) ? GJX_OK : GJX_ERR_UNSUPPORTED;
}

static int smc_plan_interp_tables(gjx_smc_plan* plan) {
  std::lock_guard<std::mutex> lock(plan->mu);
  if (plan->dev_init && plan->dev_step) return GJX_OK;
  CSite* di = nullptr; CSite* ds = nullptr;
  if (hipMalloc((void**)&di, sizeof(CSite) * (size_t)plan->n_init) != hipSuccess) return GJX_ERR_LAUNCH;
  if (hipMalloc((void**)&ds, sizeof(CSite) * (size_t)plan->n_step) != hipSuccess) { (void)hipFree(di); return GJX_ERR_LAUNCH; }
  if (hipMemcpy(di, plan->init, sizeof(CSite) * (size_t)plan->n_init, hipMemcpyHostToDevice) != hipSuccess ||
      hipMemcpy(ds, plan->step, sizeof(CSite) * (size_t)plan->n_step, hipMemcpyHostToDevice) != hipSuccess) {
    (void)hipFree(di); (void)hipFree(ds);
    return GJX_ERR_LAUNCH;
  }
  plan->dev_init = di; plan->dev_step = ds;
  return GJX_OK;
}
static gjx_jit::CompiledSmc* smc_plan_compiled(gjx_smc_plan* plan, int impl, bool peers = false) {
  if (!gjx_jit::enabled()) return nullptr;
  gjx_jit::CompiledSmc& c = peers ? plan->jit_peers[impl] : plan->jit[impl];
  const bool ready = compiled_once(plan->mu, c, {{plan->init, plan->n_init}, {plan->step, plan->n_step}}, &plan->dev_owned, [&] {
    return c.load(smc_plan_source(plan, impl, &c.tabs, peers), gjx_jit::PlanKind::smc, {"gjx_smc_step_kernel", "gjx_smc_step_kernel_adaptive", "gjx_smc_init_kernel"},
                  {&c.step, &c.step_adaptive, &c.init});
  });
  return ready ? &c : nullptr;
}

static int smc_plan_route(gjx_smc_plan* plan, int impl, gjx_jit::CompiledSmc** c_out, bool peers = false) {
  *c_out = smc_plan_compiled(plan, impl, peers);
  if (*c_out) return GJX_OK;
  if (peers) return gjx_jit::enabled() ? GJX_ERR_JIT : GJX_ERR_UNSUPPORTED;
  const bool off = !gjx_jit::enabled();
  if (!off && !jit_fallback_allowed()) return GJX_ERR_JIT;
  if (plan->has_expr || plan->guided || plan->n_params > 0 || plan->init_scopes.n_scopes > 0 || plan->step_scopes.n_scopes > 0) return off ? GJX_ERR_UNSUPPORTED : GJX_ERR_JIT;
  return smc_plan_interp_tables(plan);
}
static int smc_plan_step(const gjx_smc_config* cfg, gjx_smc_plan* plan, gjx_jit::CompiledSmc* cp, int t,
                         const float* obs_t, const gjx_smc_pop* prev, const gjx_smc_pop* out, int32_t* prev_e_out,
                         uint64_t* prev_q_out, int32_t* ancestors_out, gjx_stream s, const StepCtx& ctx,
                         const CsmcRet* ret = nullptr) {
  const bool ad = cfg_adaptive(cfg);
// ... 1665 lines not shown
```

### genjax-chi_amd/csrc/gjx_plan_jit.hpp

```cpp
#pragma once
#include <hip/hiprtc.h>

#include <atomic>
#include <cstdio>
#include <cstdlib>
#include <initializer_list>
#include <mutex>
#include <sstream>
#include <string>
#include <unordered_map>
#include <cstring>
#include <utility>
#include <vector>

#include <dirent.h>
#include <dlfcn.h>
#include <spawn.h>
#include <sys/wait.h>
#include <unistd.h>
#include <cerrno>

extern "C" char** environ;

namespace gjx_jit {
// ... 19 lines not shown
  }
  gjx::PlanTables tables() const {
    gjx::PlanTables t;
    std::memset(&t, 0, sizeof t);
    for (size_t i = 0; i < ptrs.size(); ++i) t.p[i] = ptrs[i];
    return t;
  }
};
inline TableReg*& active_tables() {
  static thread_local TableReg* reg = nullptr;
  return reg;
}
struct TableScope {
  TableReg reg;
  TableReg* prev;
  TableScope() : prev(active_tables()) { active_tables() = &reg; }
  ~TableScope() { active_tables() = prev; }
};
inline std::string plit_as(const char* type, const void* p) {
  char b[96];
  const int k = active_tables() ? active_tables()->index_of(p) : -1;
  if (k >= 0) std::snprintf(b, sizeof b, "((const %s*)tabs.p[%d])", type, k);
  else std::snprintf(b, sizeof b, "((const %s*)0x%llxull)", type, (unsigned long long)(uintptr_t)p);
  return b;
}
inline std::string plit(const void* p) { return plit_as("float", p); }

inline bool sampled_mode(int observed) { return observed == 0 || observed == GJX_SITE_PROPOSED; }
struct ScopeInfo {
  int n_scopes = 0;
  int site_scope[GJX_MAX_SITES];
  uint32_t fold_t[GJX_MAX_SITES], fold_p[GJX_MAX_SITES];
  int parent[GJX_MAX_SCOPES + 1], begin[GJX_MAX_SCOPES + 1], end[GJX_MAX_SCOPES + 1];
  uint32_t s_fold_t[GJX_MAX_SCOPES + 1], s_fold_p[GJX_MAX_SCOPES + 1];
};
inline bool derive_scopes(const gjx_site* sites, int n_sites, const gjx_scope* sc, int n_sc, ScopeInfo& out) {
  if (n_sc < 0 || n_sc > GJX_MAX_SCOPES || (n_sc && !sc)) return false;
  struct Frame { int id, end; uint32_t ct, dr; };
  Frame fr[8];
  int depth = 0, next = 0;
  fr[depth++] = Frame{0, n_sites, 1u, 0u};
  out.n_scopes = n_sc;
  out.parent[0] = -1;
  for (int q = 0; q <= n_sites; ++q) {
    while (next < n_sc && sc[next].begin == q) {
      const gjx_scope& k = sc[next];
      if (k.parent < 0 || k.parent > next || k.end < k.begin || k.end > n_sites) return false;
      while (depth > 0 && fr[depth - 1].id != k.parent) {
        if (fr[depth - 1].end > q) return false;
        --depth;
      }
      if (depth == 0 || k.end > fr[depth - 1].end || depth >= 5) return false;
      out.parent[next + 1] = k.parent;
      out.begin[next + 1] = k.begin;
      out.end[next + 1] = k.end;
      out.s_fold_t[next + 1] = fr[depth - 1].ct++;
      out.s_fold_p[next + 1] = fr[depth - 1].dr++;
      fr[depth++] = Frame{next + 1, k.end, 1u, 0u};
      ++next;
    }
    if (next < n_sc && sc[next].begin < q) return false;
    while (depth > 1 && fr[depth - 1].end <= q) --depth;
    if (q == n_sites) break;
    out.site_scope[q] = fr[depth - 1].id;
    out.fold_t[q] = fr[depth - 1].ct++;
    out.fold_p[q] = fr[depth - 1].dr;
    if (sampled_mode(sites[q].observed)) fr[depth - 1].dr++;
  }
  return next == n_sc;
}

template <class CSiteT, class CArgT>
struct SiteEmitter {
  std::ostringstream& o;
  int impl, mode;
  const CSiteT* sites;
  int n_sites;
  const char* ind;
  std::string sfx = "";
  int cur_blk = -1;
  bool store_values = true;
  bool ext_bits = false;
  bool exact_cuts = true;
  const ScopeInfo* sc = nullptr;
  const int* ret_comp = nullptr;
  bool retained(int q) const { return ret_comp && ret_comp[q] >= 0 && sampled(sites[q]); }

  int scope_of(int q) const { return sc ? sc->site_scope[q] : 0; }
  std::string key_of_scope(int k) const { return k == 0 ? "pkey" + sfx : "skey" + std::to_string(k) + sfx; }
  std::string key_of(int q) const { return key_of_scope(scope_of(q)); }
  void emit_scope_keys() {
    if (!sc) return;
    for (int k = 1; k <= sc->n_scopes; ++k)
      o << ind << "const Key " << key_of_scope(k) << " = fold_in<" << impl << ">(" << key_of_scope(sc->parent[k]) << ", "
        << (impl == 0 ? sc->s_fold_t[k] : sc->s_fold_p[k]) << "u); (void)" << key_of_scope(k) << ";\n";
    for (int k = 1; k <= sc->n_scopes; ++k) o << ind << "float " << acc("w", k) << " = 0.0f, " << acc("sc", k) << " = 0.0f;\n";
  }

  static bool is_int(const CSiteT& s) { return s.dist >= GJX_DIST_BERNOULLI; }
  static bool sampled(const CSiteT& s) { return sampled_mode(s.observed); }
  static bool proposed(const CSiteT& s) { return s.observed == GJX_SITE_PROPOSED; }
  static bool guided(const CSiteT& s) { return s.observed == GJX_SITE_GUIDED; }
  std::string nm(const char* base, int q) const { return std::string(base) + std::to_string(q) + sfx; }
  std::string val_f32(int site) const { return is_int(sites[site]) ? "(float)" + nm("vi", site) : nm("vf", site); }
  std::string val_i32(int site) const {
    return is_int(sites[site]) ? nm("vi", site) : "(int32_t)__builtin_rintf(" + nm("vf", site) + ")";
  }
  std::string arg(const CArgT& a) const {
    switch (a.kind) {
      case GJX_ARG_CONST: return flit(a.offset);
      case GJX_ARG_SITE: return "((" + flit(a.scale) + " * " + val_f32(a.ref_site) + ") + " + flit(a.offset) + ")";
      case GJX_ARG_INPUT:
        return "((" + flit(a.scale) + " * cols.in[" + std::to_string(a.ref) + "][li" + sfx + "]) + " + flit(a.offset) + ")";
      case GJX_ARG_STATE: return "((" + flit(a.scale) + " * st_" + std::to_string(a.ref) + sfx + ") + " + flit(a.offset) + ")";
      case GJX_ARG_OBS: return "((" + flit(a.scale) + " * a.obs[" + std::to_string(a.ref) + "]) + " + flit(a.offset) + ")";
      case GJX_ARG_DATA: return "((" + flit(a.scale) + " * dc" + std::to_string(a.ref) + ") + " + flit(a.offset) + ")";
      case GJX_ARG_PARAM:
        if (mode == 1 && a.scale == 1.0f && a.offset == 0.0f) return "prm.p[" + std::to_string(a.ref) + "]";
        return "((" + flit(a.scale) + " * prm.p[" + std::to_string(a.ref) + "]) + " + flit(a.offset) + ")";
      case GJX_ARG_EXPR: {
        const gjx_expr_op* ops = reinterpret_cast<const gjx_expr_op*>(a.table);
        std::vector<std::string> st;
        for (int k = 0; k < a.ref; ++k) {
          const std::string r = std::to_string(ops[k].ref);
          switch (ops[k].op) {
            case GJX_EXPR_CONST: st.push_back(flit(ops[k].value)); break;
            case GJX_EXPR_SITE: st.push_back(val_f32(ops[k].ref)); break;
            case GJX_EXPR_INPUT: st.push_back("cols.in[" + r + "][li" + sfx + "]"); break;
            case GJX_EXPR_PARAM: st.push_back("prm.p[" + r + "]"); break;
            case GJX_EXPR_STATE: st.push_back("st_" + r + sfx); break;
            case GJX_EXPR_OBS: st.push_back("a.obs[" + r + "]"); break;
            case GJX_EXPR_DATA: st.push_back("dc" + r); break;
            case GJX_EXPR_NEG: st.back() = "(-" + st.back() + ")"; break;
            case GJX_EXPR_EXP: st.back() = "e_exp(" + st.back() + ")"; break;
            case GJX_EXPR_LOG: st.back() = "m_log(" + st.back() + ")"; break;
            case GJX_EXPR_SQRT: st.back() = "__builtin_sqrtf(" + st.back() + ")"; break;
            case GJX_EXPR_ABS: st.back() = "__builtin_fabsf(" + st.back() + ")"; break;
            case GJX_EXPR_LT: case GJX_EXPR_LE: case GJX_EXPR_EQ: {
              const std::string b = st.back();
              st.pop_back();
              const char* op = ops[k].op == GJX_EXPR_LT ? " < " : (ops[k].op == GJX_EXPR_LE ? " <= " : " == ");
              st.back() = "((" + st.back() + op + b + ") ? 1.0f : 0.0f)";
              break;
            }
            case GJX_EXPR_SELECT: {
              const std::string f = st.back();
              st.pop_back();
              const std::string t = st.back();
              st.pop_back();
              st.back() = "((" + st.back() + " != 0.0f) ? " + t + " : " + f + ")";
              break;
            }
            case GJX_EXPR_MAX: case GJX_EXPR_MIN: {
              const std::string b = st.back();
              st.pop_back();
              st.back() = std::string(ops[k].op == GJX_EXPR_MAX ? "e_max(" : "e_min(") + st.back() + ", " + b + ")";
              break;
            }
            default: {
              const std::string b = st.back();
              st.pop_back();
              const char* op = ops[k].op == GJX_EXPR_ADD ? " + " : (ops[k].op == GJX_EXPR_SUB ? " - " : (ops[k].op == GJX_EXPR_MUL ? " * " : " / "));
              st.back() = "(" + st.back() + op + b + ")";
            }
          }
        }
        return st.back();
      }
      default: return plit(a.table) + "[" + val_i32(a.ref_site) + "]";
    }
  }
  bool needs_pk() const {
    for (int q = 0; q < n_sites; ++q)
      if (sampled(sites[q])) return true;
    return false;
  }
  bool needs_stream_key() const {
    for (int q = 0; q < n_sites; ++q)
      if (sampled(sites[q]) && !one_word(sites[q])) return true;
    return false;
  }
  uint32_t fold_of(int q) const {
    if (sc) return impl == 0 ? sc->fold_t[q] : sc->fold_p[q];
    if (impl == 0) return (uint32_t)(q + 1);
    uint32_t d = 0;
    for (int p = 0; p < q; ++p) d += sampled(sites[p]) ? 1u : 0u;
    return d;
  }
  bool one_word(const CSiteT& st) const {
    return st.dist == GJX_DIST_NORMAL || st.dist == GJX_DIST_BERNOULLI ||
           (st.dist == GJX_DIST_CATEGORICAL && st.cat_mode == 1);
  }
  bool pairs_normals() const { return impl == 1 && mode != 1; }

// ... 14 lines not shown
      auto carg = [&](const CArgT& a, int which) {
        float v = a.offset;
        if (a.kind == GJX_ARG_EXPR) {
          const gjx_expr_op* ops = reinterpret_cast<const gjx_expr_op*>(a.table);
          float stk[8];
          int d = 0;
          for (int k = 0; k < a.ref; ++k) {
            if ((ops[k].op >= GJX_EXPR_SITE && ops[k].op <= GJX_EXPR_OBS) || ops[k].op == GJX_EXPR_DATA) return arg(a);
            if (ops[k].op == GJX_EXPR_CONST) { stk[d++] = ops[k].value; continue; }
            if (ops[k].op == GJX_EXPR_NEG) { stk[d - 1] = -stk[d - 1]; continue; }
            if (ops[k].op == GJX_EXPR_EXP) { stk[d - 1] = gjx::e_exp(stk[d - 1]); continue; }
            if (ops[k].op == GJX_EXPR_LOG) { stk[d - 1] = gjx::m_log(stk[d - 1]); continue; }
            if (ops[k].op == GJX_EXPR_SQRT) { stk[d - 1] = __builtin_sqrtf(stk[d - 1]); continue; }
            if (ops[k].op == GJX_EXPR_ABS) { stk[d - 1] = __builtin_fabsf(stk[d - 1]); continue; }
            if (ops[k].op == GJX_EXPR_SELECT) { const float r = stk[d - 3] != 0.0f ? stk[d - 2] : stk[d - 1]; d -= 2; stk[d - 1] = r; continue; }
            if (ops[k].op == GJX_EXPR_LT || ops[k].op == GJX_EXPR_LE || ops[k].op == GJX_EXPR_EQ) {
              const float y = stk[--d], x = stk[d - 1];
              stk[d - 1] = (ops[k].op == GJX_EXPR_LT ? x < y : (ops[k].op == GJX_EXPR_LE ? x <= y : x == y)) ? 1.0f : 0.0f;
              continue;
            }
            const float y = stk[--d], x = stk[d - 1];
            stk[d - 1] = ops[k].op == GJX_EXPR_ADD ? x + y : ops[k].op == GJX_EXPR_SUB ? x - y : ops[k].op == GJX_EXPR_MUL ? x * y
                         : ops[k].op == GJX_EXPR_MAX ? gjx::e_max(x, y) : ops[k].op == GJX_EXPR_MIN ? gjx::e_min(x, y) : x / y;
          }
          v = stk[0];
        } else if (a.kind != GJX_ARG_CONST) {
          return arg(a);
        }
        bool ok = v - v == 0.0f;
        if (st.dist == GJX_DIST_NORMAL) ok = ok && (which == 0 || v > 0.0f);
        else if (st.dist == GJX_DIST_BERNOULLI) ok = ok && v >= 0.0f && v <= 1.0f;
        else ok = ok && v > 0.0f;
        if (a.kind == GJX_ARG_EXPR) return ok ? arg(a) : "opq(" + arg(a) + ")";
        return ok ? flit(v) : flit_opaque(v);
      };
      o << ind << "const float a0_" << Q << " = " << carg(st.a0, 0) << ";\n";
      if (st.dist != GJX_DIST_BERNOULLI) o << ind << "const float a1_" << Q << " = " << carg(st.a1, 1) << ";\n";
    }
    if (guided(st)) {
      if (is_int(st)) o << ind << "const int32_t vi" << Q << " = " << val_i32(st.obs.ref_site) << ";\n";
      else o << ind << "const float vf" << Q << " = " << val_f32(st.obs.ref_site) << ";\n";
      return;
    }
    if (st.observed == 1) {
      std::string ov;
      if (st.obs.kind == GJX_ARG_CONST) {
        const float v = st.obs.offset;
        const bool in_support = st.dist == GJX_DIST_GAMMA ? v > 0.0f : (st.dist == GJX_DIST_BETA ? (v > 0.0f && v < 1.0f) : true);
        ov = in_support ? flit(v) : flit_opaque(v);
      }
      else if (st.obs.kind == GJX_ARG_OBS) ov = "a.obs[" + std::to_string(st.obs.ref) + "]";
      else if (st.obs.kind == GJX_ARG_NEXT) ov = "nx_" + std::to_string(st.obs.ref);
      else if (st.obs.kind == GJX_ARG_PARAM || st.obs.kind == GJX_ARG_DATA || st.obs.kind == GJX_ARG_EXPR) ov = arg(st.obs);
      else ov = "cols.in[" + std::to_string(st.obs.ref) + "][li" + sfx + "]";
      if (is_int(st)) o << ind << "const int32_t vi" << Q << " = (int32_t)__builtin_rintf(" << ov << ");\n";
      else o << ind << "const float vf" << Q << " = " << ov << ";\n";
      return;
    }
    if (!one_word(st) || (ext_bits && scope_of(q) == 0)) return;
    if (impl == 1) {
      o << ind << "const uint32_t bits" << Q << " = philox_single_draw(" << key_of(q) << ", " << fold << "u);\n";
    } else {
      o << ind << "const uint32_t bits" << Q << " = Stream<0>(" << key_of(q) << ", true, " << fold << "u).bits32(0);\n";
    }
  }

  static bool beta_plain_ratio(const CSiteT& st) {
    return (st.a0.kind == GJX_ARG_CONST && !(st.a0.offset < 1.0f)) || (st.a1.kind == GJX_ARG_CONST && !(st.a1.offset < 1.0f));
  }

  bool presampled = false;
  bool defer_acc = false;
  void tail(int q, const std::string& eps = "") {
    const CSiteT& st = sites[q];
    const std::string I = std::to_string(impl), Q = std::to_string(q) + sfx, K = key_of(q);
    const uint32_t fold = fold_of(q);
    const std::string row = "row" + Q;
    const bool isint = is_int(st);
    const std::string VF = (retained(q) ? "vd" : "vf") + Q, VI = (retained(q) ? "vj" : "vi") + Q;
    if (sampled(st) && !(presampled && (st.dist == GJX_DIST_GAMMA || st.dist == GJX_DIST_BETA))) {
      switch (st.dist) {
        case GJX_DIST_NORMAL: {
          std::string e = eps;
          if (e.empty())
            e = pairs_normals() ? "site_normal<1>(Stream<1>(" + K + ", true, " + std::to_string(fold) + "u))"
                                : "std_normal(bits" + Q + ")";
          o << ind << "const float t" << Q << " = a1_" << Q << " * " << e << ";\n";
          o << ind << "const float " << VF << " = a0_" << Q << " + t" << Q << ";\n";
          break;
        }
        case GJX_DIST_BERNOULLI:
          o << ind << "const int32_t " << VI << " = uniform01(bits" << Q << ") < a0_" << Q << " ? 1 : 0;\n";
          break;
        case GJX_DIST_GAMMA:
          o << ind << "const Stream<" << I << "> strm" << Q << "(" << K << ", true, " << fold << "u);\n";
          o << ind << "const float " << VF << " = std_gamma<" << I << ">(strm" << Q << ", 0, a0_" << Q << ") / a1_" << Q << ";\n";
          break;
        case GJX_DIST_BETA:
          o << ind << "const Stream<" << I << "> strm" << Q << "(" << K << ", true, " << fold << "u);\n";
          o << ind << "const float g1_" << Q << " = std_gamma<" << I << ">(strm" << Q << ", 0, a0_" << Q << ");\n";
          o << ind << "const float g2_" << Q << " = std_gamma<" << I << ">(strm" << Q << ", 1, a1_" << Q << ");\n";
          if (beta_plain_ratio(st))
            o << ind << "const float " << VF << " = g1_" << Q << " / (g1_" << Q << " + g2_" << Q << ");\n";
          else
            o << ind << "const float " << VF << " = beta_from_gammas<" << I << ">(strm" << Q << ", a0_" << Q << ", a1_" << Q << ", g1_" << Q << ", g2_" << Q << ");\n";
          break;
        default:
          if (st.cat_mode == 0) {
            o << ind << "const Stream<" << I << "> strm" << Q << "(" << K << ", true, " << fold << "u);\n";
            o << ind << "const int32_t " << VI << " = jcat_gumbel<" << I << ">(" << row << ", " << st.n_cat << "u, strm" << Q << ");\n";
          } else if (st.cat_ent) {
            o << ind << "uint32_t lpb" << Q << ";\n";
            o << ind << "const int32_t " << VI << " = jcat_invcdf_gb(" << plit_as("uint4", st.cat_guide4) << " + ((size_t)rr" << Q << " << " << st.cat_gbits << "), "
              << plit_as("uint2", st.cat_ent) << " + (size_t)rr" << Q << " * " << st.n_cat << ", " << st.n_cat << "u, bits" << Q << ", " << (32 - st.cat_gbits) << ", lpb" << Q << ");\n";
          } else {
            o << ind << "const int32_t " << VI << " = jcat_invcdf(" << row << ", " << st.n_cat << "u, bits" << Q << ");\n";
          }
      }
      if (retained(q)) {
        const std::string rv = "rv_" + std::to_string(ret_comp[q]);
        if (isint) o << ind << "const int32_t vi" << Q << " = rsel" << sfx << " ? (int32_t)__builtin_rintf(__builtin_fminf(__builtin_fmaxf(" << rv << ", -1073741824.0f), 1073741824.0f)) : " << VI << ";\n";
        else o << ind << "const float vf" << Q << " = rsel" << sfx << " ? " << rv << " : " << VF << ";\n";
      }
    }
    if (defer_acc) return;
    const std::string lp = lp_of(q);
    const std::string v = (isint ? "vi" : "vf") + Q;
    const std::string aw = acc("w", scope_of(q)), as = acc("sc", scope_of(q));
    if (proposed(st)) {
      o << ind << "const float lq" << Q << " = " << lp << ";\n";
    } else if (guided(st)) {
      o << ind << "{ const float lp = " << lp << "; " << as << " = " << as << " + lp; const float d = lp - " << nm("lq", st.obs.ref_site)
        << "; " << aw << " = " << aw << " + d; }\n";
    } else {
      o << ind << "{ const float lp = " << lp << "; " << as << " = " << as << " + lp;"
        << (st.observed ? " " + aw + " = " + aw + " + lp;" : "") << " }\n";
    }
    if ((mode == 0 || mode == 2) && st.out_col >= 0 && store_values)
      o << ind << "reinterpret_cast<uint32_t*>(cols.out[" << st.out_col << "])[" << (mode == 2 ? "oi" : "i") << sfx << "] = "
        << (isint ? "(uint32_t)" + v : "f2u(" + v + ")") << ";\n";
  }
  bool normal_exact_cuts(const CSiteT& st) const {
    if (!exact_cuts || st.dist != GJX_DIST_NORMAL || st.pre != 1) return false;
    const uint32_t rs = gjx::f2u(st.pre0);
    const bool pow2 = (rs & 0x807fffffu) == 0u && rs >= 0x3f800000u && rs < 0x7f800000u;
    return pow2 && st.pre1 - st.pre1 == 0.0f && __builtin_fabsf(st.pre1) >= 7.8886090522101181e-31f;
  }
  std::string lp_of(int q) const {
    const CSiteT& st = sites[q];
    const std::string Q = std::to_string(q) + sfx;
    const std::string row = "row" + Q;
    const bool isint = is_int(st);
    std::string lp;
    const std::string v = (isint ? "vi" : "vf") + Q;
    const std::string p0 = st.pre == 2 ? "prm.d[" + std::to_string(2 * q) + "]" : flit(st.pre0);
    const std::string p1 = st.pre == 2 ? "prm.d[" + std::to_string(2 * q + 1) + "]" : flit(st.pre1);
    switch (st.dist) {
      case GJX_DIST_NORMAL:
        lp = st.pre ? "logpdf_normal_pre(" + v + ", a0_" + Q + ", " + p0 + ", " + p1 + (normal_exact_cuts(st) ? ", NormalExactCuts())" : ")")
                    : "logpdf_normal(" + v + ", a0_" + Q + ", a1_" + Q + ")";
        break;
      case GJX_DIST_GAMMA:
        lp = st.pre ? "logpdf_gamma_pre(" + v + ", a0_" + Q + ", a1_" + Q + ", " + p1 + ")"
                    : "logpdf_gamma(" + v + ", a0_" + Q + ", a1_" + Q + ")";
        break;
      case GJX_DIST_BETA:
        lp = st.pre ? "logpdf_beta_pre(" + v + ", a0_" + Q + ", a1_" + Q + ", " + p1 + ")"
                    : "logpdf_beta(" + v + ", a0_" + Q + ", a1_" + Q + ")";
        break;
      case GJX_DIST_BERNOULLI: lp = "logpdf_bernoulli(" + v + " != 0, a0_" + Q + ")"; break;
      default:
        const bool lpb_drawn = st.cat_ent && sampled(st) && st.cat_mode != 0;
        if (lpb_drawn && !retained(q))
          lp = "u2f(lpb" + Q + ")";
        else
          lp = std::string(lpb_drawn ? "(!rsel" + sfx + " ? u2f(lpb" + Q + ") : " : "") + "((" + v + " < 0 || " + v + " >= " + std::to_string(st.n_cat) + ") ? -__builtin_inff() : " +
               (st.cat_logp_t ? plit(st.cat_logp_t) + "[(size_t)" + v + " * " + std::to_string(st.n_rows) + " + rr" + Q + "]"
                : st.cat_ent ? "u2f(" + plit_as("uint2", st.cat_ent) + "[(size_t)rr" + Q + " * " + std::to_string(st.n_cat) + " + " + v + "].y)"
                             : row + "[" + v + "] - jrow_lse(" + row + ", " + std::to_string(st.n_cat) + "u)") + ")" + (lpb_drawn ? ")" : "");
    }
    auto is_const = [](const CArgT& a) {
      if (a.kind == GJX_ARG_CONST) return true;
      if (a.kind != GJX_ARG_EXPR) return false;
      const gjx_expr_op* ops = reinterpret_cast<const gjx_expr_op*>(a.table);
      for (int k = 0; k < a.ref; ++k)
        if ((ops[k].op >= GJX_EXPR_SITE && ops[k].op <= GJX_EXPR_OBS) || ops[k].op == GJX_EXPR_DATA) return false;
      return true;
    };
    const bool all_const = st.observed == 1 && st.obs.kind == GJX_ARG_CONST && is_const(st.a0) &&
                           (st.dist == GJX_DIST_BERNOULLI || st.dist == GJX_DIST_CATEGORICAL || is_const(st.a1));
    if (all_const) lp = "opq(" + lp + ")";
    return lp;
  }

  std::string acc(const char* base, int k) const { return k == 0 ? std::string(base) + sfx : std::string(base) + "_s" + std::to_string(k) + sfx; }
  void close_scopes(int pos) {
    if (!sc) return;
    for (int k = sc->n_scopes; k >= 1; --k)
      if (sc->end[k] == pos && sc->begin[k] < pos)
        o << ind << acc("w", sc->parent[k]) << " = " << acc("w", sc->parent[k]) << " + " << acc("w", k) << "; "
          << acc("sc", sc->parent[k]) << " = " << acc("sc", sc->parent[k]) << " + " << acc("sc", k) << ";\n";
  }
  void run() {
    emit_scope_keys();
    for (int q = 0; q < n_sites; ++q) {
      head(q);
      tail(q);
      close_scopes(q + 1);
    }
  }
};

inline void emit_prelude(std::ostringstream& o, bool fast_math = false, bool bm_lds = false, int block = 0) {
  if (bm_lds) o << "#define GJX_BM_LDS 1\n#define GJX_BM_BLOCK " << block << "\n";
  if (fast_math) o << "#define GJX_FAST_MATH 1\n";
  o << "#include \"gjx_device.hpp\"\nusing namespace gjx;\n";
}

template <class CSiteT, class CArgT>
inline void emit_pair_lane_sites(std::ostringstream& o, std::vector<SiteEmitter<CSiteT, CArgT>>& em, const CSiteT* sites, int n_sites,
                                 int NP, const std::string& ind, const std::string& store_at, const std::string& sc_guard = "",
                                 const std::string& ubase = "", const std::string& lane_bytes = "") {
  const char* sfx[4] = {"A", "B", "C", "D"};
  const int P = 2 * NP;
int cur_pair_blk = -1;
  for (int q = 0; q < n_sites; ++q) {
    const CSiteT& st = sites[q];
    const bool pinned = !sc_guard.empty() && em[0].scope_of(q) == 0;
    for (int u = 0; u < P; ++u) em[u].defer_acc = pinned;
    for (int u = 0; u < P; ++u) em[u].head(q);
    const std::string Q = std::to_string(q);
    if (!st.observed && em[0].one_word(st) && em[0].scope_of(q) == 0) {
      const uint32_t f = em[0].fold_of(q);
      const int blk = (int)(f >> 1);
      const std::string B = std::to_string(blk);
      if (blk != cur_pair_blk) {
        cur_pair_blk = blk;
        for (int pi = 0; pi < NP; ++pi) {
          const std::string V = "pp" + std::to_string(pi) + "_" + B;
          o << ind << "uint32_t " << V << "_0, " << V << "_1, " << V << "_2, " << V << "_3;\n";
          o << ind << "philox4x32(pk0, pk1, (uint32_t)pair" << pi << ", (uint32_t)(pair" << pi << " >> 32), " << blk << "u, kTagPair, " << V
            << "_0, " << V << "_1, " << V << "_2, " << V << "_3);\n";
        }
      }
      for (int pi = 0; pi < NP; ++pi) {
        const std::string V = "pp" + std::to_string(pi) + "_" + B;
        o << ind << "const uint32_t bits" << Q << sfx[2 * pi] << " = " << V << "_" << ((f & 1u) << 1) << ", bits" << Q << sfx[2 * pi + 1]
          << " = " << V << "_" << (((f & 1u) << 1) | 1u) << ";\n";
      }
    }
    if (!st.observed && st.dist == GJX_DIST_NORMAL && em[0].scope_of(q) == 0) {
      for (int pi = 0; pi < NP; ++pi) {
        const std::string Z = Q + "_" + std::to_string(pi);
        o << ind << "float zc" << Z << ", zs" << Z << ";\n      bm_pair(bits" << Q << sfx[2 * pi] << ", bits" << Q << sfx[2 * pi + 1] << ", zc" << Z
          << ", zs" << Z << ");\n";
      }
      for (int pi = 0; pi < NP; ++pi) {
        const std::string Z = Q + "_" + std::to_string(pi);
        em[2 * pi].tail(q, "zc" + Z);
        em[2 * pi + 1].tail(q, "zs" + Z);
      }
    } else if (!st.observed && (st.dist == GJX_DIST_GAMMA || st.dist == GJX_DIST_BETA)) {
      const std::string I = std::to_string(em[0].impl), PS = std::to_string(P);
      const uint32_t fold = em[0].fold_of(q);
      o << ind << "float vg0_" << Q << "[" << PS << "]" << (st.dist == GJX_DIST_BETA ? ", vg1_" + Q + "[" + PS + "]" : std::string()) << ";\n";
      o << ind << "{\n" << ind << "  const Stream<" << I << "> gs[" << PS << "] = {";
      for (int u = 0; u < P; ++u) o << (u ? ", " : "") << "Stream<" << I << ">(" << em[u].key_of(q) << ", true, " << fold << "u)";
      o << "};\n";
      o << ind << "  const float gc0[" << PS << "] = {";
      for (int u = 0; u < P; ++u) o << (u ? ", " : "") << "a0_" << Q << sfx[u];
      o << "};\n" << ind << "  std_gamma_multi<" << I << ", " << PS << ">(gs, 0, gc0, vg0_" << Q << ");\n";
      if (st.dist == GJX_DIST_BETA) {
        o << ind << "  const float gc1[" << PS << "] = {";
        for (int u = 0; u < P; ++u) o << (u ? ", " : "") << "a1_" << Q << sfx[u];
        o << "};\n" << ind << "  std_gamma_multi<" << I << ", " << PS << ">(gs, 1, gc1, vg1_" << Q << ");\n";
      }
      o << ind << "}\n";
      for (int u = 0; u < P; ++u) {
        if (st.dist == GJX_DIST_GAMMA)
          o << ind << "const float vf" << Q << sfx[u] << " = vg0_" << Q << "[" << u << "] / a1_" << Q << sfx[u] << ";\n";
        else if (em[0].beta_plain_ratio(st))
          o << ind << "const float vf" << Q << sfx[u] << " = vg0_" << Q << "[" << u << "] / (vg0_" << Q << "[" << u << "] + vg1_" << Q << "[" << u << "]);\n";
        else
          o << ind << "const float vf" << Q << sfx[u] << " = beta_from_gammas<" << I << ">(Stream<" << I << ">(" << em[u].key_of(q) << ", true, " << fold
            << "u), a0_" << Q << sfx[u] << ", a1_" << Q << sfx[u] << ", vg0_" << Q << "[" << u << "], vg1_" << Q << "[" << u << "]);\n";
        em[u].presampled = true;
        em[u].tail(q);
        em[u].presampled = false;
      }
    } else {
      for (int u = 0; u < P; ++u) em[u].tail(q);
    }
    if (pinned) {
      auto pins = [&](const char* base) {
        std::string t;
        for (int pi = 0; pi < NP; ++pi) {
          const std::string a = std::string(base) + sfx[2 * pi], b = std::string(base) + sfx[2 * pi + 1];
          t += " { const pin2_t t = pinned2(" + a + ", " + b + "); " + a + " = t[0]; " + b + " = t[1]; }";
        }
        return t;
      };
      if (st.observed) {
        for (int u = 0; u < P; ++u) o << ind << "const float lp" << Q << sfx[u] << " = " << em[u].lp_of(q) << ";\n";
        o << ind;
        for (int u = 0; u < P; ++u) o << "w" << sfx[u] << " = w" << sfx[u] << " + lp" << Q << sfx[u] << "; ";
        o << pins("w") << "\n";
        o << ind << "if (" << sc_guard << ") { ";
        for (int u = 0; u < P; ++u) o << "sc" << sfx[u] << " = sc" << sfx[u] << " + lp" << Q << sfx[u] << "; ";
        o << pins("sc") << " }\n";
      } else {
        o << ind << "if (" << sc_guard << ") {\n";
        for (int u = 0; u < P; ++u)
          o << ind << "  { const float lp = " << em[u].lp_of(q) << "; sc" << sfx[u] << " = sc" << sfx[u] << " + lp; }\n";
        o << ind << " " << pins("sc") << "\n" << ind << "}\n";
      }
      for (int u = 0; u < P; ++u) em[u].defer_acc = false;
    }
    for (int u = 0; u < P; ++u) em[u].close_scopes(q + 1);
    if (st.out_col >= 0) {
      const bool isint = SiteEmitter<CSiteT, CArgT>::is_int(st);
      std::string vals;
      for (int u = 0; u < P; ++u)
        vals += (u ? ", " : "") + (isint ? "(uint32_t)vi" + Q + sfx[u] : "f2u(vf" + Q + sfx[u] + ")");
      if (P == 4 && !ubase.empty())
        o << ind << "store16_at(reinterpret_cast<uint32_t*>(cols.out[" << st.out_col << "]) + " << ubase << ", " << lane_bytes << ", make_uint4(" << vals << "), wt_one_pass);\n";
      else if (P == 4)
        o << ind << "store16_out(reinterpret_cast<uint32_t*>(cols.out[" << st.out_col << "]) + " << store_at << ", make_uint4(" << vals << "), wt_one_pass);\n";
      else
        o << ind << "*reinterpret_cast<uint" << P << "*>(reinterpret_cast<uint32_t*>(cols.out[" << st.out_col << "]) + " << store_at << ") = make_uint" << P
          << "(" << vals << ");\n";
    }
  }
}

template <class CSiteT, class CArgT>
struct Gen {
  std::ostringstream o;
  int impl;
  const CSiteT* sites;
  int n_sites;
  int min_waves = 0;
  bool fused_tail = false;
  bool wt_stores = false;
  int block = 256;
  int rows_per_block = 1;
  bool laned = false;
  bool fast_math = false;
  const ScopeInfo* sc = nullptr;
  int pairs_per_lane = 1;

  static const char* signature() {
    return "(KeySrc ks, RunCols cols, float* score, float* logw, uint64_t n, float* max_partials, int32_t* row_e, "
           "uint64_t* row_s, LseTail tail, PassBatch bt, PlanParams prm, PlanTables tabs) {\n";
  }
  const char* kname() const { return impl == 0 ? "gjx_plan_kernel_threefry" : "gjx_plan_kernel_philox"; }
  bool bm_lds() const {
    if (impl != 1 || fast_math) return false;
    for (int q = 0; q < n_sites; ++q)
      if (!sites[q].observed && sites[q].dist == GJX_DIST_NORMAL) return true;
    return false;
  }
  std::string bounds(int threads) const { return "__launch_bounds__(" + std::to_string(threads) + ", GJX_WAVES_HINT)"; }
  void emit_hint_default() { o << "#ifndef GJX_WAVES_HINT\n#define GJX_WAVES_HINT " << (min_waves > 0 ? min_waves : 0) << "\n#endif\n"; }
  const char* tail_scope() const { return fused_tail ? "tail.tickets != nullptr" : "false"; }
  void emit_tail() {
    o << "  }\n";
    if (fused_tail) o << "  if (row_e) lse_tail(row_e, row_s, (n + 255) / 256, tail, blockIdx.y * gridDim.x + blockIdx.x, gridDim.x * gridDim.y);\n";
    o << "}\n";
  }
  void emit_pass_key() {
    o << "  const uint32_t pass = blockIdx.y, grid_x = gridDim.x;  // (pass < bt.n_pass <= kMaxPasses: the host launches n_pass rows of workgroups)\n";
    o << "  const uint32_t bk0 = bt.parent[pass][0], bk1 = bt.parent[pass][1];\n";
  }

  std::string run_paired() {
    const int NP = pairs_per_lane == 2 ? 2 : 1;
    const int lanes_per_row = 128 / NP;
    bool any_col = false;
    for (int q = 0; q < n_sites; ++q) any_col = any_col || sites[q].out_col >= 0;
    const int R = (NP == 2 && !any_col) ? 4 : 1;
    block = lanes_per_row * R;
    rows_per_block = R;
    const int waves_per_row = lanes_per_row / 64;
    const bool ubase = NP == 2 && R == 1;
    emit_prelude(o, fast_math, bm_lds(), block);
    emit_hint_default();
    o << "extern \"C\" __global__ " << bounds(block) << " void " << kname() << signature();
    if (waves_per_row > 1) o << "  __shared__ float sh_red[" << waves_per_row * R << "];\n  __shared__ uint64_t sh_sum[" << waves_per_row * R << "];\n";
    if (R == 1) o << "  const int wv = threadIdx.x >> 6, pr = 0, tr = threadIdx.x;  // (block-uniform row: the cipher key stays scalar)\n";
    else o << "  const int wv = threadIdx.x >> 6, pr = threadIdx.x / " << lanes_per_row << ", tr = threadIdx.x % " << lanes_per_row << ";\n";
    o << "  (void)wv;\n";
    if (bm_lds()) o << "  const BmLoads bm_loads = bm_issue();\n";
    emit_pass_key();
    o << "  asm volatile(\"\" :: \"s\"(n), \"s\"(score), \"s\"(logw), \"s\"(max_partials), \"s\"(row_e), \"s\"(row_s), \"s\"(bt.n_pass), \"s\"(bt.rows_per_pass), \"s\"(bt.pass_stride), \"s\"(bt.row_stride), \"s\"(ks.first), \"s\"(ks.parent.k0), \"s\"(ks.parent.k1), \"s\"(bk0), \"s\"(bk1), \"s\"(grid_x)"
      << (fused_tail ? ", \"s\"(tail.tickets)" : "") << ");\n";
    {
      bool seen[64] = {};
      for (int q = 0; q < n_sites; ++q)
        if (sites[q].out_col >= 0 && sites[q].out_col < 64 && !seen[sites[q].out_col]) {
          seen[sites[q].out_col] = true;
          o << "  asm volatile(\"\" :: \"s\"(cols.out[" << sites[q].out_col << "]));\n";
        }
    }
    if (bm_lds()) o << "  bm_loads.bm_stage();\n";
    o << "  const bool wt_one_pass = " << (wt_stores ? "true" : "false") << "; (void)wt_one_pass;  // (Gen::wt_stores)\n";
    o << "  const uint32_t pk0 = bt.n_pass > 1 ? bk0 : ks.parent.k0, pk1 = bt.n_pass > 1 ? bk1 : ks.parent.k1;\n";
    o << "  const uint64_t po = (uint64_t)pass * bt.pass_stride, ro = (uint64_t)pass * bt.row_stride;  // this pass's outputs\n";
    o << "  for (uint64_t g0 = (uint64_t)blockIdx.x * " << R << "; g0 < bt.rows_per_pass; g0 += (uint64_t)grid_x * " << R << ") {\n";
    o << "    const uint64_t row = g0 + pr;\n";
    o << "    const bool live_row = row < bt.rows_per_pass;  // (the four-row workgroup: the dead rows at the end of a pass)\n";
    o << "    uint64_t rrow = ro + row;\n";
    if (NP == 2 && R == 1) o << "    asm volatile(\"\" : \"+s\"(rrow));\n";
    const char* sfx[4] = {"A", "B", "C", "D"};
    const int P = 2 * NP;
    o << "    const uint64_t iA = row * 256 + " << P << " * (uint64_t)tr;\n";
    for (int u = 1; u < P; ++u) o << "    const uint64_t i" << sfx[u] << " = iA + " << u << ";\n";
    o << "    const bool ok = live_row && iA < n;\n";
    if (ubase) o << "    const uint64_t ub = po + row * 256;\n    uint32_t lb = 16u * (uint32_t)tr;\n    asm volatile(\"\" : \"+v\"(lb));\n";
    for (int u = 0; u < P; ++u) o << "    const uint64_t li" << sfx[u] << " = i" << sfx[u] << "; (void)li" << sfx[u] << ";\n";
    for (int u = 0; u < P; ++u) o << "    float w" << sfx[u] << " = 0.0f, sc" << sfx[u] << " = 0.0f;\n";
    o << "    if (ok) {\n";
    o << "      const uint64_t lnA = ks.first + iA + 1u;\n";
    for (int u = 0; u < P; ++u) {
      if (u) o << "      const uint64_t ln" << sfx[u] << " = lnA + " << u << "u;\n";
      o << "      const Key pkey" << sfx[u] << "{pk0, pk1, (uint32_t)ln" << sfx[u] << ", (uint32_t)(ln" << sfx[u] << " >> 32)}; (void)pkey" << sfx[u] << ";\n";
    }
    std::vector<SiteEmitter<CSiteT, CArgT>> em;
    for (int u = 0; u < P; ++u) {
      em.push_back(SiteEmitter<CSiteT, CArgT>{o, impl, 0, sites, n_sites, "      ", sfx[u]});
      em.back().store_values = false;
      em.back().ext_bits = true;
      em.back().sc = sc;
    }
    for (int u = 0; u < P; ++u) em[u].emit_scope_keys();
    o << "      const uint64_t pair0 = (lnA - 1u) >> 1;\n";
    if (NP == 2) o << "      const uint64_t pair1 = pair0 + 1u;\n";
    emit_pair_lane_sites<CSiteT, CArgT>(o, em, sites, n_sites, NP, "      ", "po + iA", "score", ubase ? "ub" : "", "lb");
    if (ubase) {
      std::string wb, sb;
      for (int u = 0; u < P; ++u) { wb += (u ? ", f2u(w" : "f2u(w") + std::string(sfx[u]) + ")"; sb += (u ? ", f2u(sc" : "f2u(sc") + std::string(sfx[u]) + ")"; }
      o << "      if (logw) store16_at(logw + ub, lb, make_uint4(" << wb << "), wt_one_pass);\n";
      o << "      if (score) store16_at(score + ub, lb, make_uint4(" << sb << "), wt_one_pass);\n";
    } else if (P == 4) {
      std::string wb, sb;
      for (int u = 0; u < P; ++u) { wb += (u ? ", f2u(w" : "f2u(w") + std::string(sfx[u]) + ")"; sb += (u ? ", f2u(sc" : "f2u(sc") + std::string(sfx[u]) + ")"; }
      o << "      if (logw) store16_out(logw + po + iA, make_uint4(" << wb << "), wt_one_pass);\n";
      o << "      if (score) store16_out(score + po + iA, make_uint4(" << sb << "), wt_one_pass);\n";
    } else {
      std::string ws, ss;
      for (int u = 0; u < P; ++u) { ws += (u ? ", w" : "w") + std::string(sfx[u]); ss += (u ? ", sc" : "sc") + std::string(sfx[u]); }
      o << "      if (logw) *reinterpret_cast<float" << P << "*>(logw + po + iA) = make_float" << P << "(" << ws << ");\n";
      o << "      if (score) *reinterpret_cast<float" << P << "*>(score + po + iA) = make_float" << P << "(" << ss << ");\n";
    }
    o << "    }\n";
    o << "    if (max_partials || row_e) {\n";
    o << "      const float ninf = -__builtin_inff();\n";
    {
      std::string mx = "wA";
      for (int u = 1; u < P; ++u) mx = "(" + mx + " > w" + sfx[u] + " ? " + mx + " : w" + sfx[u] + ")";
      o << "      float bm = wave_max(ok ? " << mx << " : ninf);\n";
    }
    if (waves_per_row > 1) {
      o << "      __syncthreads();\n      if ((threadIdx.x & 63) == 0) sh_red[wv] = bm;\n      __syncthreads();\n";
      o << "      bm = sh_red[2 * pr] > sh_red[2 * pr + 1] ? sh_red[2 * pr] : sh_red[2 * pr + 1];\n";
    }
    const char* lane0 = ubase ? "lb == 0u" : "tr == 0";
    o << "      if (max_partials && " << lane0 << " && live_row) max_partials[rrow] = bm;\n";
    o << "      if (row_e) {\n";
    o << "        const int32_t eb = row_anchor(bm);\n";
    {
      std::string sm;
      for (int u = 0; u < P; ++u) sm += (u ? " + rowfix(w" : "rowfix(w") + std::string(sfx[u]) + ", eb)";
      o << "        uint64_t sb = wave_sum_52(ok ? (" << sm << ") : 0);  // (at most four weights below 2^32)\n";
    }
    if (waves_per_row > 1) {
      o << "        __syncthreads();\n        if ((threadIdx.x & 63) == 0) sh_sum[wv] = sb;\n        __syncthreads();\n";
      o << "        sb = sh_sum[2 * pr] + sh_sum[2 * pr + 1];\n";
    }
    o << "        if (" << lane0 << " && live_row) lse_store_row(row_e, row_s, rrow, eb, sb, " << tail_scope() << ");\n";
    o << "      }\n    }\n";
    emit_tail();
    return o.str();
  }

  std::string run() {
    if (laned && impl == 1) return run_paired();
    const std::string I = std::to_string(impl);
    emit_prelude(o, fast_math, bm_lds(), 256);
    emit_hint_default();
    o << "extern \"C\" __global__ " << bounds(256) << " void " << kname() << signature();
    o << "  __shared__ float sh_red[4];\n  __shared__ uint64_t sh_sum[4];\n";
    emit_pass_key();
    o << "  asm volatile(\"\" :: \"s\"(bk0), \"s\"(bk1), \"s\"(grid_x));\n";
    if (bm_lds()) o << "  bm_stage();\n";
    o << "  const uint64_t po = (uint64_t)pass * bt.pass_stride, ro = (uint64_t)pass * bt.row_stride;\n";
    o << "  KeySrc kp = ks;\n";
    o << "  if (bt.n_pass > 1) { kp.parent.k0 = bk0; kp.parent.k1 = bk1; }\n";
    o << "  for (uint64_t row = blockIdx.x; row < bt.rows_per_pass; row += grid_x) {\n";
    o << "    float tmax = -__builtin_inff();\n    bool live = false;\n";
    o << "    {\n";
    o << "      const uint64_t li = row * 256 + threadIdx.x, i = po + li;\n";
    o << "      const bool ok = li < n;\n";
    o << "      if (ok) {\n";
    o << "        const Key pkey = key_at<" << I << ">(kp, li);\n";
    o << "        float w = 0.0f, sc = 0.0f;\n";
    SiteEmitter<CSiteT, CArgT> em{o, impl, 0, sites, n_sites, "        "};
    em.sc = sc;
    em.run();
    o << "        if (logw) logw[i] = w;\n        if (score) score[i] = sc;\n        tmax = w;\n        live = true;\n";
    o << "      }\n    }\n";
    o << "    if (max_partials || row_e) {\n";
    o << "      const float bm = block_max(tmax, sh_red);\n";
    o << "      if (max_partials && threadIdx.x == 0) max_partials[ro + row] = bm;\n";
    o << "      if (row_e) {\n";
    o << "        const int32_t eb = row_anchor(bm);\n";
    o << "        const uint64_t sb = block_sum(live ? rowfix(tmax, eb) : 0, sh_sum);\n";
    o << "        if (threadIdx.x == 0) lse_store_row(row_e, row_s, ro + row, eb, sb, " << tail_scope() << ");\n";
    o << "      }\n    }\n";
    emit_tail();
    return o.str();
  }
};

template <class CSiteT, class CArgT>
struct GenScan {
  std::ostringstream o;
  int impl;
  const CSiteT* sites;
  int n_sites;
  const CArgT* next_state;
  int n_state, n_obs;
  bool fast_math = false;
  const ScopeInfo* sc = nullptr;
  bool quad = false;
  int block = 256;
  bool fused_tail = false;
  const char* tail_scope() const { return fused_tail ? "tail.tickets != nullptr" : "false"; }
  void emit_tail() {
    o << "  }\n";
    if (fused_tail) o << "  if (row_e) lse_tail(row_e, row_s, (n + 255) / 256, tail, blockIdx.x, gridDim.x);\n";
    o << "}\n";
  }
  const char* kname() const { return impl == 0 ? "gjx_scan_kernel_threefry" : "gjx_scan_kernel_philox"; }
  bool bm_lds() const {
    if (impl != 1 || fast_math) return false;
    for (int q = 0; q < n_sites; ++q)
      if (!sites[q].observed && sites[q].dist == GJX_DIST_NORMAL) return true;
    return false;
  }
  std::string run_quad() {
    block = 64;
    const char* sfx[4] = {"A", "B", "C", "D"};
    const int P = 4;
    emit_prelude(o, fast_math, bm_lds(), block);
    o << "struct StepObs { const float* obs; };\n";
    o << "extern \"C\" __global__ __launch_bounds__(64) void " << kname()
      << "(KeySrc ks, RunCols cols, ScanArgs sa, float* score, float* logw, float* max_partials, int32_t* row_e, uint64_t* row_s, LseTail tail, PlanTables tabs) {\n";
    if (bm_lds()) o << "  bm_stage();\n";
    o << "  const uint64_t n = sa.n, rows_all = (n + 255) / 256;\n";
    o << "  const bool wt_one_pass = false; (void)wt_one_pass;  // (a scan's stores spread over its T steps)\n";
    o << "  const uint32_t pk0 = ks.parent.k0, pk1 = ks.parent.k1;\n";
    o << "  for (uint64_t row = blockIdx.x; row < rows_all; row += gridDim.x) {\n";
    o << "    const uint64_t iA = row * 256 + 4 * (uint64_t)threadIdx.x;\n";
    o << "    const bool ok = iA < n;  // (n is a multiple of four in this form: all particles of a lane exist or none)\n";
    for (int u = 0; u < P; ++u) o << "    float wt" << sfx[u] << " = 0.0f, sct" << sfx[u] << " = 0.0f;\n";
    o << "    if (ok) {\n";
    o << "      const uint64_t lnA = ks.first + iA + 1u;\n";
    for (int u = 0; u < P; ++u)
      for (int k = 0; k < n_state; ++k)
        o << "      float st_" << k << sfx[u] << " = sa.carry0_cols[" << k << "] ? sa.carry0_cols[" << k << "][iA + " << u << "] : sa.carry0[" << k << "];\n";
    o << "      for (int32_t t = 0; t < sa.n_steps; ++t) {\n";
    o << "        const uint64_t lt = lnA + (((uint64_t)(uint32_t)t + 1u) << 40);  // the lanes of step t (scan_step_key_philox)\n";
    for (int u = 0; u < P; ++u)
      o << "        const Key pkey" << sfx[u] << "{pk0, pk1, (uint32_t)(lt + " << u << "u), (uint32_t)((lt + " << u << "u) >> 32)}; (void)pkey" << sfx[u] << ";\n";
    o << "        const uint64_t pair0 = (lt - 1u) >> 1, pair1 = pair0 + 1u;\n";
    o << "        StepObs a; a.obs = sa.obs + (size_t)t * " << n_obs << "; (void)a;\n";
    o << "        const uint64_t oiA = (uint64_t)t * sa.col_stride + iA; (void)oiA;\n";
    for (int u = 0; u < P; ++u) o << "        float w" << sfx[u] << " = 0.0f, sc" << sfx[u] << " = 0.0f;\n";
    std::vector<SiteEmitter<CSiteT, CArgT>> em;
    for (int u = 0; u < P; ++u) {
      em.push_back(SiteEmitter<CSiteT, CArgT>{o, impl, 2, sites, n_sites, "        ", sfx[u]});
      em.back().store_values = false;
      em.back().ext_bits = true;
      em.back().sc = sc;
    }
    for (int u = 0; u < P; ++u) em[u].emit_scope_keys();
    emit_pair_lane_sites<CSiteT, CArgT>(o, em, sites, n_sites, 2, "        ", "oiA");
    for (int u = 0; u < P; ++u)
      for (int k = 0; k < n_state; ++k) o << "        const float nx_" << k << sfx[u] << " = " << em[u].arg(next_state[k]) << ";\n";
    for (int u = 0; u < P; ++u)
      for (int k = 0; k < n_state; ++k) o << "        st_" << k << sfx[u] << " = nx_" << k << sfx[u] << ";\n";
    for (int u = 0; u < P; ++u) o << "        wt" << sfx[u] << " = wt" << sfx[u] << " + w" << sfx[u] << "; sct" << sfx[u] << " = sct" << sfx[u] << " + sc" << sfx[u] << ";\n";
    o << "      }\n";
    for (int k = 0; k < n_state; ++k)
      o << "      if (sa.carry_out[" << k << "]) *reinterpret_cast<float4*>(sa.carry_out[" << k << "] + iA) = make_float4(st_" << k << "A, st_" << k
        << "B, st_" << k << "C, st_" << k << "D);\n";
    o << "      if (logw) *reinterpret_cast<float4*>(logw + iA) = make_float4(wtA, wtB, wtC, wtD);\n";
    o << "      if (score) *reinterpret_cast<float4*>(score + iA) = make_float4(sctA, sctB, sctC, sctD);\n";
    o << "    }\n";
    o << "    if (max_partials || row_e) {\n";
    o << "      const float ninf = -__builtin_inff();\n";
    o << "      const float m4 = ((wtA > wtB ? wtA : wtB) > wtC ? (wtA > wtB ? wtA : wtB) : wtC);\n";
    o << "      const float bm = wave_max(ok ? (m4 > wtD ? m4 : wtD) : ninf);\n";
    o << "      if (max_partials && threadIdx.x == 0) max_partials[row] = bm;\n";
    o << "      if (row_e) {\n";
    o << "        const int32_t eb = row_anchor(bm);\n";
    o << "        const uint64_t sb = wave_sum(ok ? (rowfix(wtA, eb) + rowfix(wtB, eb) + rowfix(wtC, eb) + rowfix(wtD, eb)) : 0);\n";
    o << "        if (threadIdx.x == 0) lse_store_row(row_e, row_s, row, eb, sb, " << tail_scope() << ");\n";
    o << "      }\n    }\n";
    emit_tail();
    return o.str();
  }
  std::string run() {
    if (quad && impl == 1) return run_quad();
    const std::string I = std::to_string(impl);
    emit_prelude(o, fast_math, bm_lds(), 256);
    o << "struct StepObs { const float* obs; };\n";
    o << "extern \"C\" __global__ __launch_bounds__(256) void " << kname()
      << "(KeySrc ks, RunCols cols, ScanArgs sa, float* score, float* logw, float* max_partials, int32_t* row_e, uint64_t* row_s, LseTail tail, PlanTables tabs) {\n";
    o << "  __shared__ float sh_red[4];\n  __shared__ uint64_t sh_sum[4];\n";
    if (bm_lds()) o << "  bm_stage();\n";
    o << "  const uint64_t n = sa.n, rows_all = (n + 255) / 256;\n";
    o << "  for (uint64_t row = blockIdx.x; row < rows_all; row += gridDim.x) {\n";
    o << "    float tmax = -__builtin_inff();\n    bool live = false;\n";
    o << "    const uint64_t i = row * 256 + threadIdx.x;\n";
    o << "    if (i < n) {\n";
    o << "      Key " << (impl == 0 ? "pkey" : "pkey0") << " = key_at<" << I << ">(ks, i);\n";
    for (int k = 0; k < n_state; ++k)
      o << "      float st_" << k << " = sa.carry0_cols[" << k << "] ? sa.carry0_cols[" << k << "][i] : sa.carry0[" << k << "];\n";
    o << "      float wt = 0.0f, sct = 0.0f;\n";
    o << "      for (int32_t t = 0; t < sa.n_steps; ++t) {\n";
    if (impl == 0) o << "        pkey = fold_in<0>(pkey, (uint32_t)t);  // chained: the folded key is carried (scan.py:267-268)\n";
    else o << "        const Key pkey = scan_step_key_philox(pkey0, (uint32_t)t);  // a lane per (particle, step): no cipher block\n";
    o << "        StepObs a; a.obs = sa.obs + (size_t)t * " << n_obs << "; (void)a;\n";
    o << "        const uint64_t oi = (uint64_t)t * sa.col_stride + i; (void)oi;\n";
    o << "        float w = 0.0f, sc = 0.0f;\n";
    SiteEmitter<CSiteT, CArgT> em{o, impl, 2, sites, n_sites, "        "};
    em.sc = sc;
    em.run();
    for (int k = 0; k < n_state; ++k) o << "        const float nx_" << k << " = " << em.arg(next_state[k]) << ";\n";
    for (int k = 0; k < n_state; ++k) o << "        st_" << k << " = nx_" << k << ";\n";
    o << "        wt = wt + w;\n        sct = sct + sc;\n      }\n";
    for (int k = 0; k < n_state; ++k) o << "      if (sa.carry_out[" << k << "]) sa.carry_out[" << k << "][i] = st_" << k << ";\n";
    o << "      if (logw) logw[i] = wt;\n      if (score) score[i] = sct;\n      tmax = wt;\n      live = true;\n    }\n";
    o << "    if (max_partials || row_e) {\n";
    o << "      const float bm = block_max(tmax, sh_red);\n";
    o << "      if (max_partials && threadIdx.x == 0) max_partials[row] = bm;\n";
    o << "      if (row_e) {\n";
    o << "        const int32_t eb = row_anchor(bm);\n";
    o << "        const uint64_t sb = block_sum(live ? rowfix(tmax, eb) : 0, sh_sum);\n";
    o << "        if (threadIdx.x == 0) lse_store_row(row_e, row_s, row, eb, sb, " << tail_scope() << ");\n";
    o << "      }\n    }\n";
    emit_tail();
    return o.str();
  }
};

template <class CSiteT, class CArgT>
struct GenSmc {
  std::ostringstream o;
  int impl;
  const CSiteT* init_sites;
  int n_init;
  const CSiteT* step_sites;
  int n_step;
  const CArgT* init_state;
  const CArgT* next_state;
  int n_state;
  const ScopeInfo* sc_init = nullptr;
  const ScopeInfo* sc_step = nullptr;
  bool peers = false;
  int n_params = 0;
  int row_len() const { return n_params + 2 * (n_init + n_step); }
  bool cond = false;
  int ret_init[GJX_MAX_SITES], ret_step[GJX_MAX_SITES];
  static bool csmc_components(const CSiteT* sites, int n_sites, const CArgT* state, int n_state, int* comp) {
    for (int q = 0; q < n_sites; ++q) comp[q] = -1;
    for (int k = 0; k < n_state; ++k) {
      const CArgT& a = state[k];
      if (a.kind != GJX_ARG_SITE || a.scale != 1.0f || a.offset != 0.0f || a.ref_site < 0 || a.ref_site >= n_sites) return false;
      if (!sampled_mode(sites[a.ref_site].observed) || comp[a.ref_site] >= 0) return false;
      comp[a.ref_site] = k;
    }
    for (int q = 0; q < n_sites; ++q)
      if (sampled_mode(sites[q].observed) && comp[q] < 0) return false;
    return true;
// ... 814 lines not shown
```

### include/gjx.h

```cpp
#ifndef GJX_H
#define GJX_H

#include <stddef.h>
#include <stdint.h>

#ifdef __cplusplus
extern "C" {
#endif

#define GJX_VERSION_MAJOR 0
#define GJX_VERSION_MINOR 10

typedef void* gjx_stream;

typedef enum {
  GJX_OK = 0,
  GJX_ERR_INVALID = -1,
  GJX_ERR_UNSUPPORTED = -2,
  GJX_ERR_WORKSPACE = -3,
  GJX_ERR_LAUNCH = -4,
  GJX_ERR_NO_DEVICE = -5,
  GJX_ERR_JIT = -6
} gjx_status;

// ... 61 lines not shown
  GJX_DIST_CATEGORICAL = 4
} gjx_dist;

typedef enum {
  GJX_ARG_CONST = 0,
  GJX_ARG_SITE = 1,
  GJX_ARG_INPUT = 2,
  GJX_ARG_TABLE = 3,
  GJX_ARG_STATE = 4,
  GJX_ARG_OBS = 5,
  GJX_ARG_PARAM = 6,
  GJX_ARG_EXPR = 7
} gjx_arg_kind;
#define GJX_MAX_PARAMS 64

typedef enum {
  GJX_EXPR_CONST = 0,
  GJX_EXPR_SITE = 1,
  GJX_EXPR_INPUT = 2,
  GJX_EXPR_PARAM = 3,
  GJX_EXPR_STATE = 4,
  GJX_EXPR_OBS = 5,
  GJX_EXPR_ADD = 6,
  GJX_EXPR_SUB = 7,
  GJX_EXPR_MUL = 8,
  GJX_EXPR_NEG = 9,
  GJX_EXPR_DIV = 10,
  GJX_EXPR_EXP = 11,
  GJX_EXPR_LOG = 12,
  GJX_EXPR_SQRT = 13,
  GJX_EXPR_ABS = 14,
  GJX_EXPR_MAX = 15,
  GJX_EXPR_MIN = 16,
  GJX_EXPR_LT = 17,
  GJX_EXPR_LE = 18,
  GJX_EXPR_EQ = 19,
  GJX_EXPR_SELECT = 20
} gjx_expr_opcode;
typedef struct {
  int32_t op;
  int32_t ref;
  float value;
} gjx_expr_op;
#define GJX_MAX_EXPR_OPS 32

typedef struct {
  int32_t kind;
  int32_t ref;
  float scale;
  float offset;
  const float* table;
} gjx_arg;

typedef struct {
  int32_t dist;
  int32_t observed;
  int32_t out_col;
  int32_t n_cat;
  int32_t n_rows;
  int32_t cat_mode;
  gjx_arg arg[2];
  gjx_arg obs;
  const float* logits;
} gjx_site;

typedef struct gjx_plan gjx_plan;

#define GJX_MAX_SITES 64

int gjx_plan_create(const gjx_site* sites , int n_sites, gjx_plan** out);
#define GJX_PLAN_FAST_MATH 1u
int gjx_plan_create_ex(const gjx_site* sites , int n_sites, uint32_t flags, gjx_plan** out);
typedef struct {
  int32_t parent;
  int32_t begin, end;
} gjx_scope;
#define GJX_MAX_SCOPES 16
int gjx_plan_create_scoped(const gjx_site* sites , int n_sites, const gjx_scope* scopes , int n_scopes,
                           uint32_t flags, gjx_plan** out);
int gjx_plan_destroy(gjx_plan* p);
int gjx_plan_set_params(gjx_plan* p, const float* params , int n_params);
#define GJX_SOURCE_FUSED_TAIL 0x100
#define GJX_SOURCE_WT_STORES 0x200
int gjx_plan_specialized_source(const gjx_plan* p, int impl, char* buf, size_t buf_len, size_t* needed);
int gjx_plan_prepare(gjx_plan* p, const gjx_keys* particle_keys);
int gjx_plan_compile_check(const gjx_plan* p, int impl);
int gjx_jit_stats(uint64_t* compiles, uint64_t* cached_modules, uint64_t* evictions);
int gjx_jit_routes(uint64_t* child_compiles, uint64_t* inproc_compiles, uint64_t* child_failures, uint64_t* spawn_failures);
int gjx_smc_run_graph_stats(uint64_t* captures, uint64_t* replays);
int gjx_jit_compile_source(const char* source);
#define GJX_LSE_TICKET_WORDS (17 * 64)
typedef struct {
  int32_t* e;
  uint64_t* q;
  float* lse;
  uint64_t* record;
  uint32_t* tickets;
  float* lse_shifted;
  float shift;
} gjx_lse_out;
int gjx_importance_run(const gjx_plan* p, const gjx_keys* particle_keys,
                       const float* const* input_cols, int n_input_cols, void* const* value_cols,
                       int n_value_cols, float* score, float* logw, uint64_t n,
                       float* max_partials, int32_t* row_e, uint64_t* row_s, const gjx_lse_out* lse,
                       gjx_stream s);

typedef struct {
  const gjx_plan* plan;
  uint64_t n;
  const float* const* input_cols;
  int32_t n_input_cols;
  int32_t impl;
  int32_t* row_e;
  uint64_t* row_s;
  gjx_lse_out lse;
} gjx_estimate_io;
int gjx_importance_estimate(const gjx_estimate_io* io, uint32_t k0, uint32_t k1, uint64_t lane, float* out ,
                            float shift, gjx_stream s);

int gjx_importance_run_batch(const gjx_plan* p, const gjx_keys* particle_keys , int32_t n_pass,
                             uint64_t pass_stride, uint64_t row_stride, const float* const* input_cols,
                             int n_input_cols, void* const* value_cols, int n_value_cols, float* score,
                             float* logw, uint64_t n, float* max_partials, int32_t* row_e, uint64_t* row_s,
                             gjx_stream s);


typedef enum {
  GJX_OP_LOGSUMEXP = 0,
  GJX_OP_CATEGORICAL_INDEX = 1,
  GJX_OP_RESAMPLE = 2,
  GJX_OP_SMC = 3
} gjx_op;
size_t gjx_workspace_bytes(int op, uint64_t n);

int gjx_frac_bits(uint64_t n_total);

uint64_t gjx_num_tiles(uint64_t n);
uint64_t gjx_num_max_partials(uint64_t n);

#define GJX_LSE_RECORD_WORDS 65
int gjx_row_stats(const float* x, uint64_t n, int32_t* row_e, uint64_t* row_s, gjx_stream s);
int gjx_lse_rows(const int32_t* row_e, const uint64_t* row_s, uint64_t n_rows, int32_t* out_e ,
                 uint64_t* out_q , float* out_lse , uint64_t* out_record ,
                 gjx_stream s);
int gjx_lse_rows_batch(const int32_t* row_e, const uint64_t* row_s, uint64_t n_rows, int32_t n_batch,
                       uint64_t batch_stride, int32_t* out_e, uint64_t* out_q, float* out_lse,
                       uint64_t* out_record, gjx_stream s);
int gjx_lse_combine(const uint64_t* records, int32_t n_records, uint64_t record_stride, int32_t n_batch,
                    uint64_t batch_stride, int32_t* out_e, uint64_t* out_q, float* out_lse,
                    uint64_t* out_record, gjx_stream s);

int gjx_max_f32(const float* x, uint64_t n, const float* max_partials_in, float* out_max, void* ws,
                size_t ws_bytes, gjx_stream s);
int gjx_expsum_fix(const float* x, uint64_t n, const float* max_dev, int frac_bits,
                   uint64_t* out_q, void* ws, size_t ws_bytes, gjx_stream s);
int gjx_lse_finish(const float* max_dev, const uint64_t* q_dev, int frac_bits, float* out_lse,
                   gjx_stream s);
int gjx_logsumexp_f32(const float* x, uint64_t n, const float* max_partials_in, float* out_lse,
                      float* out_max, uint64_t* out_q, void* ws, size_t ws_bytes, gjx_stream s);

int gjx_categorical_index(const gjx_keys* key, const float* logits, uint64_t n, int64_t* out_idx,
                          int mode, void* ws, size_t ws_bytes, gjx_stream s);

int gjx_categorical_index_batch(const gjx_keys* keys , int32_t n_batch, const float* logits, uint64_t n,
                                uint64_t stride, int64_t* out_idx, gjx_stream s);

// ... 214 lines not shown
```

Baseline: 97.31 billion.

## Trim JIT kernel arithmetic: zero-loc normals, fused rowfix exp, ordered-int wave max

Adds several micro-optimizations to the generated importance kernel. Standard-normal sites with loc 0 and scale 1 reuse the raw noise directly and propagate as identity references. rowfix folds the 2^30 scale into the exponent shift instead of a multiply. Wave max uses a signed-integer ordered key in place of float compares. A full-outputs kernel variant drops null-pointer guards and first-accumulation adds. Each change removes a few ALU ops per particle, at the cost of more specialized variants to compile and subtle -0/NaN semantics that a new debug sweep checks.

```diff
diff --git a/genjax-chi_amd/csrc/gjx_device.hpp b/genjax-chi_amd/csrc/gjx_device.hpp
--- a/genjax-chi_amd/csrc/gjx_device.hpp
+++ b/genjax-chi_amd/csrc/gjx_device.hpp
@@ -343,7 +343,7 @@
   if (x > 88.0f) x = 88.0f;
   return m_exp_core(x);
 }
-GJX_HD float m_exp_core(float x) {
+GJX_HD float m_exp_core_shl(float x, int32_t k) {
   const float fx = __builtin_rintf(x * 1.44269504088896341f);
   x = __builtin_fmaf(fx, -0.693359375f, x);
   x = __builtin_fmaf(fx, 2.12194440e-4f, x);
@@ -356,8 +356,9 @@
   p = __builtin_fmaf(p, x, 5.0000001201E-1f);
   const float y = __builtin_fmaf(p, z, x) + 1.0f;
   const int32_t n = (int32_t)fx;
-  return u2f(f2u(y) + ((uint32_t)n << 23));
-}
+  return u2f(f2u(y) + ((uint32_t)(n + k) << 23));
+}
+GJX_HD float m_exp_core(float x) { return m_exp_core_shl(x, 0); }
 
 GJX_HD float e_exp(float x) {
   if (x != x) return x;
@@ -581,15 +582,15 @@
   return __builtin_sqrtf(x);
 #endif
 }
-GJX_HD void bm_pair(uint32_t w_radius, uint32_t w_angle, float& z_cos, float& z_sin) {
+GJX_HD void bm_parts(uint32_t w_radius, uint32_t w_angle, float& r_out, float& t_cos, float& t_sin) {
   const float uw = (float)w_radius + 1.0f;
 #ifdef GJX_FAST_MATH_DEVICE
   {
     const float u = uw * 2.3283064365386963e-10f;
-    const float rf = __builtin_amdgcn_sqrtf(-1.38629436111989062f * __builtin_amdgcn_logf(u));
+    r_out = __builtin_amdgcn_sqrtf(-1.38629436111989062f * __builtin_amdgcn_logf(u));
     const float tf = (float)(w_angle >> 8) * 5.9604644775390625e-08f;
-    z_cos = rf * __builtin_amdgcn_cosf(tf);
-    z_sin = rf * __builtin_amdgcn_sinf(tf);
+    t_cos = __builtin_amdgcn_cosf(tf);
+    t_sin = __builtin_amdgcn_sinf(tf);
     return;
   }
 #endif
@@ -609,8 +610,27 @@
   const float sd = __builtin_fmaf(d2 * d, -0.166666672f, d);
   const float cd = __builtin_fmaf(d2, __builtin_fmaf(d2, 0.0416666679f, -0.5f), 1.0f);
   const float ca = u2f(cs.a), sa = u2f(cs.b);
-  z_cos = r * __builtin_fmaf(ca, cd, -(sa * sd));
-  z_sin = r * __builtin_fmaf(sa, cd, ca * sd);
+  r_out = r;
+  t_cos = __builtin_fmaf(ca, cd, -(sa * sd));
+  t_sin = __builtin_fmaf(sa, cd, ca * sd);
+}
+GJX_HD void bm_pair(uint32_t w_radius, uint32_t w_angle, float& z_cos, float& z_sin) {
+  float r, tc, ts;
+  bm_parts(w_radius, w_angle, r, tc, ts);
+  z_cos = r * tc;
+  z_sin = r * ts;
+}
+struct PlusZero {};
+GJX_HD void bm_pair(uint32_t w_radius, uint32_t w_angle, float& z_cos, float& z_sin, PlusZero) {
+  float r, tc, ts;
+  bm_parts(w_radius, w_angle, r, tc, ts);
+#if defined(GJX_ZERO_LOC_PLAIN) || defined(GJX_FAST_MATH_DEVICE)
+  z_cos = 0.0f + r * tc;
+  z_sin = 0.0f + r * ts;
+#else
+  z_cos = __builtin_fmaf(r, tc, 0.0f);
+  z_sin = __builtin_fmaf(r, ts, 0.0f);
+#endif
 }
 constexpr uint32_t kTagTwin = 0x54u;
 template <int IMPL>
@@ -836,9 +856,15 @@
     const float fe = (float)e;
     float d = __builtin_fmaf(-fe, 0.693359375f, lw);
     d = __builtin_fmaf(-fe, -2.12194440e-4f, d);
+#if defined(GJX_ROWFIX_PLAIN) || defined(GJX_FAST_MATH_DEVICE)
     d = d > 1.0f ? 1.0f : d;
     const bool live = e != kRowEmpty && lw > -__builtin_inff() && d >= -86.0f;
     const uint32_t q = (uint32_t)__builtin_rintf(d_exp_core(live ? d : 0.0f) * 1073741824.0f);
+#else
+    d = __builtin_fminf(d, 1.0f);
+    const bool live = e != kRowEmpty && lw > -__builtin_inff() && d >= -86.0f;
+    const uint32_t q = (uint32_t)__builtin_rintf(m_exp_core_shl(live ? d : 0.0f, 30));
+#endif
     return live ? q : 0u;
   }
 #endif
@@ -983,6 +1009,26 @@
   const uint32_t r = wave_scan_u32(f2u(v), f2u(-__builtin_inff()),
                                    [](uint32_t a, uint32_t b) { return u2f(b) > u2f(a) ? b : a; });
   return u2f(wave_last_u32(r));
+}
+GJX_HD int32_t order_key(uint32_t bits) { return (int32_t)(bits ^ ((uint32_t)((int32_t)bits >> 31) & 0x7fffffffu)); }
+GJX_DEV float wave_max_ordered(float v) {
+#ifdef GJX_WAVE_MAX_SELECT
+  return wave_max(v);
+#else
+  v = v == v ? v : -__builtin_inff();
+  uint32_t mask = (uint32_t)((int32_t)f2u(v) >> 31) & 0x7fffffffu;
+  asm volatile("" : "+v"(mask));
+  const uint32_t r = wave_scan_u32(f2u(v) ^ mask, 0x80000000u,
+                                   [](uint32_t a, uint32_t b) { return (uint32_t)((int32_t)b > (int32_t)a ? (int32_t)b : (int32_t)a); });
+  return u2f((uint32_t)order_key(wave_last_u32(r)));
+#endif
+}
+GJX_HD float first_acc(float lp) {
+#ifdef GJX_FIRST_ACC_PLAIN
+  return 0.0f + lp;
+#else
+  return lp;
+#endif
 }
 GJX_DEV uint64_t wave_sum(uint64_t v) {
   return wave_last_u64(wave_scan_u64(v, 0, [](uint64_t a, uint64_t b) { return a + b; }));
diff --git a/genjax-chi_amd/csrc/gjx_hip.hip b/genjax-chi_amd/csrc/gjx_hip.hip
--- a/genjax-chi_amd/csrc/gjx_hip.hip
+++ b/genjax-chi_amd/csrc/gjx_hip.hip
@@ -1687,6 +1687,26 @@
     atomicMin(&out[1], first);
   }
 }
+__global__ __launch_bounds__(kBlock) void k_zero_loc_sweep(uint32_t wr0, uint32_t wr1, unsigned long long* out) {
+  unsigned long long bad = 0, first = ~0ull;
+  for (uint64_t i = (uint64_t)blockIdx.x * kBlock + threadIdx.x; i < ((uint64_t)1 << 24); i += (uint64_t)gridDim.x * kBlock) {
+    const uint32_t wa = (uint32_t)i << 8;
+#pragma unroll
+    for (int k = 0; k < 2; ++k) {
+      float zc, zs, pc, ps;
+      bm_pair(k ? wr1 : wr0, wa, zc, zs);
+      bm_pair(k ? wr1 : wr0, wa, pc, ps, PlusZero());
+      if (f2u(0.0f + zc) != f2u(pc) || f2u(0.0f + zs) != f2u(ps)) {
+        ++bad;
+        first = first < i ? first : i;
+      }
+    }
+  }
+  if (bad) {
+    atomicAdd(&out[0], bad);
+    atomicMin(&out[1], first);
+  }
+}
 }
 
 static int copy_source_out(const std::string& src, char* buf, size_t buf_len, size_t* needed) {
@@ -1937,6 +1957,7 @@
   gjx_jit::Compiled jit[4];
   gjx_jit::Compiled jit_tail[4];
   gjx_jit::Compiled jit_wt[2];
+  gjx_jit::Compiled jit_full[2];
   std::vector<void*> dev_owned;
   std::mutex jit_mu;
   ExprStore expr;
@@ -2184,32 +2205,36 @@
   return 4;
 }
 static int jit_waves_hint(int P) { return P == 2 ? 6 : 0; }
-static void plan_gen_setup(gjx_jit::Gen<CSite, CArg>& g, const gjx_plan* p, int impl, int form, bool fused_tail, bool wt_stores, int min_waves) {
+static void plan_gen_setup(gjx_jit::Gen<CSite, CArg>& g, const gjx_plan* p, int impl, int form, bool fused_tail, bool wt_stores, int min_waves,
+                           bool full_outputs = false) {
   g.impl = impl; g.sites = p->host; g.n_sites = p->n_sites; g.laned = form >= 2; g.pairs_per_lane = form == 4 ? 2 : 1;
   g.sc = p->scopes.n_scopes > 0 ? &p->scopes : nullptr;
   g.fast_math = (p->flags & GJX_PLAN_FAST_MATH) != 0;
   g.fused_tail = fused_tail;
   g.wt_stores = wt_stores;
+  g.full_outputs = full_outputs;
   g.min_waves = min_waves;
 }
 int gjx_plan_specialized_source(const gjx_plan* p, int impl, char* buf, size_t buf_len, size_t* needed) {
   const bool fused_tail = (impl & GJX_SOURCE_FUSED_TAIL) != 0, wt_stores = (impl & GJX_SOURCE_WT_STORES) != 0;
-  impl &= ~(GJX_SOURCE_FUSED_TAIL | GJX_SOURCE_WT_STORES);
+  const bool full_outputs = (impl & GJX_SOURCE_FULL_OUTPUTS) != 0;
+  impl &= ~(GJX_SOURCE_FUSED_TAIL | GJX_SOURCE_WT_STORES | GJX_SOURCE_FULL_OUTPUTS);
   if (!p || (impl != 0 && impl != 1)) return GJX_ERR_INVALID;
   const int form = impl == 1 ? jit_form_pref() : 1;
   gjx_jit::Gen<CSite, CArg> g;
-  plan_gen_setup(g, p, impl, form, fused_tail, wt_stores, jit_waves_hint(form));
+  plan_gen_setup(g, p, impl, form, fused_tail, wt_stores, jit_waves_hint(form), full_outputs);
   gjx_jit::TableScope ts;
   return copy_source_out(g.run(), buf, buf_len, needed);
 }
 
 int gjx_plan_compile_check(const gjx_plan* p, int impl) {
   const bool fused_tail = (impl & GJX_SOURCE_FUSED_TAIL) != 0, wt_stores = (impl & GJX_SOURCE_WT_STORES) != 0;
-  impl &= ~(GJX_SOURCE_FUSED_TAIL | GJX_SOURCE_WT_STORES);
+  const bool full_outputs = (impl & GJX_SOURCE_FULL_OUTPUTS) != 0;
+  impl &= ~(GJX_SOURCE_FUSED_TAIL | GJX_SOURCE_WT_STORES | GJX_SOURCE_FULL_OUTPUTS);
   if (!p || (impl != 0 && impl != 1)) return GJX_ERR_INVALID;
   for (int form = 1; form <= (impl == 1 ? 4 : 1); form *= 2) {
     gjx_jit::Gen<CSite, CArg> g;
-    plan_gen_setup(g, p, impl, form, fused_tail, wt_stores && form == 4, jit_waves_hint(form));
+    plan_gen_setup(g, p, impl, form, fused_tail, wt_stores && form == 4, jit_waves_hint(form), full_outputs && form == 4);
     gjx_jit::TableScope ts;
     if (!gjx_jit::compile_only(g.run(), gjx_jit::PlanKind::importance)) return GJX_ERR_UNSUPPORTED;
   }
@@ -2221,22 +2246,27 @@
   for (auto& c : p->jit) c.release();
   for (auto& c : p->jit_tail) c.release();
   for (auto& c : p->jit_wt) c.release();
+  for (auto& c : p->jit_full) c.release();
   free_owned(p->dev_owned);
   delete p;
   return GJX_OK;
 }
 
-static gjx_jit::Compiled& plan_compiled(gjx_plan* mp, const gjx_keys* pk, int lane_particles, bool fused_tail = false, bool one_pass = false) {
+static gjx_jit::Compiled& plan_compiled(gjx_plan* mp, const gjx_keys* pk, int lane_particles, bool fused_tail = false, bool one_pass = false,
+                                        bool all_outputs = false) {
   const bool pairable = pk->impl == 1 && pk->mode == 1 && pk->parent_lane == 0 && (pk->first & 1) == 0;
   int P = pairable ? (lane_particles < jit_form_pref() ? lane_particles : jit_form_pref()) : 1;
   if (P == 3) P = 2;
   const bool laned = P >= 2;
   const bool wt_stores = one_pass && P == 4;
-  gjx_jit::Compiled& c = wt_stores ? mp->jit_wt[fused_tail ? 1 : 0] : (fused_tail ? mp->jit_tail : mp->jit)[P == 4 ? 3 : (laned ? 2 : pk->impl)];
+  const bool full_outputs = all_outputs && !fused_tail && P == 4;
+  gjx_jit::Compiled& c = full_outputs ? mp->jit_full[wt_stores ? 1 : 0]
+                         : wt_stores  ? mp->jit_wt[fused_tail ? 1 : 0]
+                                      : (fused_tail ? mp->jit_tail : mp->jit)[P == 4 ? 3 : (laned ? 2 : pk->impl)];
   compiled_once(mp->jit_mu, c, {{mp->host, mp->n_sites}}, &mp->dev_owned, [&] {
     auto build = [&](int min_waves) {
       gjx_jit::Gen<CSite, CArg> g;
-      plan_gen_setup(g, mp, pk->impl, P, fused_tail, wt_stores, min_waves);
+      plan_gen_setup(g, mp, pk->impl, P, fused_tail, wt_stores, min_waves, full_outputs);
       gjx_jit::TableScope ts;
       const std::string src = g.run();
       c.block = g.block;
@@ -2249,7 +2279,8 @@
     if (ok && std::getenv("GJX_PLAN_JIT_VERBOSE")) {
       int regs = 0;
       if (hipFuncGetAttribute(&regs, HIP_FUNC_ATTRIBUTE_NUM_REGS, c.fn) != hipSuccess) (void)hipGetLastError();
-      fprintf(stderr, "gjx jit: %d particle(s) per lane%s%s: %d registers per lane\n", P, fused_tail ? ", fused tail" : "", wt_stores ? ", write-through stores" : "", regs);
+      fprintf(stderr, "gjx jit: %d particle(s) per lane%s%s%s: %d registers per lane\n", P, fused_tail ? ", fused tail" : "", wt_stores ? ", write-through stores" : "",
+              full_outputs ? ", every output" : "", regs);
     }
     if (ok && hint > 0) {
       int scratch = 0;
@@ -2284,6 +2315,8 @@
   ok = plan_compiled(p, pk, 2).state == 1 && ok;
   ok = plan_compiled(p, pk, 4).state == 1 && ok;
   ok = plan_compiled(p, pk, 4, false, true).state == 1 && ok;
+  ok = plan_compiled(p, pk, 4, false, false, true).state == 1 && ok;
+  ok = plan_compiled(p, pk, 4, false, true, true).state == 1 && ok;
   if (ok) return GJX_OK;
   return jit_fallback_allowed() && !p->has_expr ? plan_device_table(p) : GJX_ERR_JIT;
 }
@@ -2333,7 +2366,8 @@
     uintptr_t al = (uintptr_t)logw | (uintptr_t)score | (uintptr_t)(4 * pass_stride) | (uintptr_t)(4 * n);
     for (int c = 0; c < n_value_cols; ++c) al |= (uintptr_t)value_cols[c];
     const int lane_particles = (al & 15) == 0 ? 4 : ((al & 7) == 0 ? 2 : 1);
-    gjx_jit::Compiled& c = plan_compiled(const_cast<gjx_plan*>(p), pk, lane_particles, lse != nullptr, n_pass <= 1);
+    const bool all_outputs = score && logw && max_partials && row_e && row_s && !lse;
+    gjx_jit::Compiled& c = plan_compiled(const_cast<gjx_plan*>(p), pk, lane_particles, lse != nullptr, n_pass <= 1, all_outputs);
     if (c.state != 1 && (!jit_fallback_allowed() || p->has_expr || p->scopes.n_scopes > 0)) return GJX_ERR_JIT;
     if (c.state == 1) {
       uint64_t nn = n;
@@ -3394,6 +3428,11 @@
   const uint64_t count = (uint64_t)hi_bits - lo_bits + 1;
   const uint64_t blocks = (count + kBlock - 1) / kBlock;
   k_sqrt_pos_sweep<<<(unsigned)(blocks < 2048 ? blocks : 2048), kBlock, 0, S(s)>>>(lo_bits, count, reinterpret_cast<unsigned long long*>(out));
+  return launch_status();
+}
+int gjx_debug_zero_loc_sweep(uint32_t w_radius0, uint32_t w_radius1, uint64_t* out, gjx_stream s) {
+  if (!out) return GJX_ERR_INVALID;
+  k_zero_loc_sweep<<<2048, kBlock, 0, S(s)>>>(w_radius0, w_radius1, reinterpret_cast<unsigned long long*>(out));
   return launch_status();
 }
 int gjx_jit_stats(uint64_t* compiles, uint64_t* cached_modules, uint64_t* evictions) {
diff --git a/genjax-chi_amd/csrc/gjx_plan_jit.hpp b/genjax-chi_amd/csrc/gjx_plan_jit.hpp
--- a/genjax-chi_amd/csrc/gjx_plan_jit.hpp
+++ b/genjax-chi_amd/csrc/gjx_plan_jit.hpp
@@ -125,7 +125,17 @@
   bool store_values = true;
   bool ext_bits = false;
   bool exact_cuts = true;
+  bool row_cuts = false;
   const ScopeInfo* sc = nullptr;
+  bool zero_loc_unit(int q) const {
+    const CSiteT& st = sites[q];
+    return row_cuts && pairs_normals() && st.dist == GJX_DIST_NORMAL && st.observed == 0 && scope_of(q) == 0 && !retained(q) &&
+           st.a0.kind == GJX_ARG_CONST && gjx::f2u(st.a0.offset) == 0u && st.a1.kind == GJX_ARG_CONST && st.a1.offset == 1.0f;
+  }
+  bool identity_ref(const CArgT& a) const {
+    return a.kind == GJX_ARG_SITE && a.scale == 1.0f && gjx::f2u(a.offset) == 0u && a.ref_site >= 0 && a.ref_site < n_sites &&
+           zero_loc_unit(a.ref_site);
+  }
   const int* ret_comp = nullptr;
   bool retained(int q) const { return ret_comp && ret_comp[q] >= 0 && sampled(sites[q]); }
 
@@ -152,7 +162,9 @@
   std::string arg(const CArgT& a) const {
     switch (a.kind) {
       case GJX_ARG_CONST: return flit(a.offset);
-      case GJX_ARG_SITE: return "((" + flit(a.scale) + " * " + val_f32(a.ref_site) + ") + " + flit(a.offset) + ")";
+      case GJX_ARG_SITE:
+        if (identity_ref(a)) return nm("vf", a.ref_site);
+        return "((" + flit(a.scale) + " * " + val_f32(a.ref_site) + ") + " + flit(a.offset) + ")";
       case GJX_ARG_INPUT:
         return "((" + flit(a.scale) + " * cols.in[" + std::to_string(a.ref) + "][li" + sfx + "]) + " + flit(a.offset) + ")";
       case GJX_ARG_STATE: return "((" + flit(a.scale) + " * st_" + std::to_string(a.ref) + sfx + ") + " + flit(a.offset) + ")";
@@ -333,6 +345,10 @@
       switch (st.dist) {
         case GJX_DIST_NORMAL: {
           std::string e = eps;
+          if (zero_loc_unit(q)) {
+            o << ind << "const float " << VF << " = " << e << ";\n";
+            break;
+          }
           if (e.empty())
             e = pairs_normals() ? "site_normal<1>(Stream<1>(" + K + ", true, " + std::to_string(fold) + "u))"
                                 : "std_normal(bits" + Q + ")";
@@ -471,10 +487,12 @@
 template <class CSiteT, class CArgT>
 inline void emit_pair_lane_sites(std::ostringstream& o, std::vector<SiteEmitter<CSiteT, CArgT>>& em, const CSiteT* sites, int n_sites,
                                  int NP, const std::string& ind, const std::string& store_at, const std::string& sc_guard = "",
-                                 const std::string& ubase = "", const std::string& lane_bytes = "") {
+                                 const std::string& ubase = "", const std::string& lane_bytes = "", bool sc_known = false) {
   const char* sfx[4] = {"A", "B", "C", "D"};
   const int P = 2 * NP;
-int cur_pair_blk = -1;
+  int cur_pair_blk = -1;
+  const std::string if_sc = sc_known ? "" : "if (" + sc_guard + ") ";
+  bool w_open = false, sc_open = false;
   for (int q = 0; q < n_sites; ++q) {
     const CSiteT& st = sites[q];
     const bool pinned = !sc_guard.empty() && em[0].scope_of(q) == 0;
@@ -504,7 +522,7 @@
       for (int pi = 0; pi < NP; ++pi) {
         const std::string Z = Q + "_" + std::to_string(pi);
         o << ind << "float zc" << Z << ", zs" << Z << ";\n      bm_pair(bits" << Q << sfx[2 * pi] << ", bits" << Q << sfx[2 * pi + 1] << ", zc" << Z
-          << ", zs" << Z << ");\n";
+          << ", zs" << Z << (em[0].zero_loc_unit(q) ? ", PlusZero());\n" : ");\n");
       }
       for (int pi = 0; pi < NP; ++pi) {
         const std::string Z = Q + "_" + std::to_string(pi);
@@ -551,20 +569,27 @@
         }
         return t;
       };
+      const bool never_neg_zero = em[0].row_cuts && !em[0].sc && st.observed <= 1 && em[0].normal_exact_cuts(st);
+      auto acc_to = [&](const char* base, bool first, int u, const std::string& lp) {
+        const std::string a = std::string(base) + sfx[u];
+        return first ? a + " = first_acc(" + lp + "); " : a + " = " + a + " + " + lp + "; ";
+      };
       if (st.observed) {
         for (int u = 0; u < P; ++u) o << ind << "const float lp" << Q << sfx[u] << " = " << em[u].lp_of(q) << ";\n";
         o << ind;
-        for (int u = 0; u < P; ++u) o << "w" << sfx[u] << " = w" << sfx[u] << " + lp" << Q << sfx[u] << "; ";
+        for (int u = 0; u < P; ++u) o << acc_to("w", !w_open && never_neg_zero, u, "lp" + Q + sfx[u]);
         o << pins("w") << "\n";
-        o << ind << "if (" << sc_guard << ") { ";
-        for (int u = 0; u < P; ++u) o << "sc" << sfx[u] << " = sc" << sfx[u] << " + lp" << Q << sfx[u] << "; ";
+        o << ind << if_sc << "{ ";
+        for (int u = 0; u < P; ++u) o << acc_to("sc", !sc_open && never_neg_zero, u, "lp" + Q + sfx[u]);
         o << pins("sc") << " }\n";
+        w_open = true;
       } else {
-        o << ind << "if (" << sc_guard << ") {\n";
+        o << ind << if_sc << "{\n";
         for (int u = 0; u < P; ++u)
-          o << ind << "  { const float lp = " << em[u].lp_of(q) << "; sc" << sfx[u] << " = sc" << sfx[u] << " + lp; }\n";
+          o << ind << "  { const float lp = " << em[u].lp_of(q) << "; " << acc_to("sc", !sc_open && never_neg_zero, u, "lp") << "}\n";
         o << ind << " " << pins("sc") << "\n" << ind << "}\n";
       }
+      sc_open = true;
       for (int u = 0; u < P; ++u) em[u].defer_acc = false;
     }
     for (int u = 0; u < P; ++u) em[u].close_scopes(q + 1);
@@ -593,6 +618,7 @@
   int min_waves = 0;
   bool fused_tail = false;
   bool wt_stores = false;
+  bool full_outputs = false;
   int block = 256;
   int rows_per_block = 1;
   bool laned = false;
@@ -634,6 +660,7 @@
     rows_per_block = R;
     const int waves_per_row = lanes_per_row / 64;
     const bool ubase = NP == 2 && R == 1;
+    const bool full = full_outputs && ubase;
     emit_prelude(o, fast_math, bm_lds(), block);
     emit_hint_default();
     o << "extern \"C\" __global__ " << bounds(block) << " void " << kname() << signature();
@@ -681,17 +708,18 @@
       em.push_back(SiteEmitter<CSiteT, CArgT>{o, impl, 0, sites, n_sites, "      ", sfx[u]});
       em.back().store_values = false;
       em.back().ext_bits = true;
+      em.back().row_cuts = true;
       em.back().sc = sc;
     }
     for (int u = 0; u < P; ++u) em[u].emit_scope_keys();
     o << "      const uint64_t pair0 = (lnA - 1u) >> 1;\n";
     if (NP == 2) o << "      const uint64_t pair1 = pair0 + 1u;\n";
-    emit_pair_lane_sites<CSiteT, CArgT>(o, em, sites, n_sites, NP, "      ", "po + iA", "score", ubase ? "ub" : "", "lb");
+    emit_pair_lane_sites<CSiteT, CArgT>(o, em, sites, n_sites, NP, "      ", "po + iA", "score", ubase ? "ub" : "", "lb", full);
     if (ubase) {
       std::string wb, sb;
       for (int u = 0; u < P; ++u) { wb += (u ? ", f2u(w" : "f2u(w") + std::string(sfx[u]) + ")"; sb += (u ? ", f2u(sc" : "f2u(sc") + std::string(sfx[u]) + ")"; }
-      o << "      if (logw) store16_at(logw + ub, lb, make_uint4(" << wb << "), wt_one_pass);\n";
-      o << "      if (score) store16_at(score + ub, lb, make_uint4(" << sb << "), wt_one_pass);\n";
+      o << "      " << (full ? "" : "if (logw) ") << "store16_at(logw + ub, lb, make_uint4(" << wb << "), wt_one_pass);\n";
+      o << "      " << (full ? "" : "if (score) ") << "store16_at(score + ub, lb, make_uint4(" << sb << "), wt_one_pass);\n";
     } else if (P == 4) {
       std::string wb, sb;
       for (int u = 0; u < P; ++u) { wb += (u ? ", f2u(w" : "f2u(w") + std::string(sfx[u]) + ")"; sb += (u ? ", f2u(sc" : "f2u(sc") + std::string(sfx[u]) + ")"; }
@@ -704,20 +732,20 @@
       o << "      if (score) *reinterpret_cast<float" << P << "*>(score + po + iA) = make_float" << P << "(" << ss << ");\n";
     }
     o << "    }\n";
-    o << "    if (max_partials || row_e) {\n";
+    o << "    " << (full ? "" : "if (max_partials || row_e) ") << "{\n";
     o << "      const float ninf = -__builtin_inff();\n";
     {
       std::string mx = "wA";
       for (int u = 1; u < P; ++u) mx = "(" + mx + " > w" + sfx[u] + " ? " + mx + " : w" + sfx[u] + ")";
-      o << "      float bm = wave_max(ok ? " << mx << " : ninf);\n";
+      o << "      float bm = " << (waves_per_row == 1 ? "wave_max_ordered" : "wave_max") << "(ok ? " << mx << " : ninf);\n";
     }
     if (waves_per_row > 1) {
       o << "      __syncthreads();\n      if ((threadIdx.x & 63) == 0) sh_red[wv] = bm;\n      __syncthreads();\n";
       o << "      bm = sh_red[2 * pr] > sh_red[2 * pr + 1] ? sh_red[2 * pr] : sh_red[2 * pr + 1];\n";
     }
     const char* lane0 = ubase ? "lb == 0u" : "tr == 0";
-    o << "      if (max_partials && " << lane0 << " && live_row) max_partials[rrow] = bm;\n";
-    o << "      if (row_e) {\n";
+    o << "      if (" << (full ? "" : "max_partials && ") << lane0 << " && live_row) max_partials[rrow] = bm;\n";
+    o << "      " << (full ? "" : "if (row_e) ") << "{\n";
     o << "        const int32_t eb = row_anchor(bm);\n";
     {
       std::string sm;
@@ -833,6 +861,7 @@
       em.push_back(SiteEmitter<CSiteT, CArgT>{o, impl, 2, sites, n_sites, "        ", sfx[u]});
       em.back().store_values = false;
       em.back().ext_bits = true;
+      em.back().row_cuts = true;
       em.back().sc = sc;
     }
     for (int u = 0; u < P; ++u) em[u].emit_scope_keys();
@@ -852,7 +881,7 @@
     o << "    if (max_partials || row_e) {\n";
     o << "      const float ninf = -__builtin_inff();\n";
     o << "      const float m4 = ((wtA > wtB ? wtA : wtB) > wtC ? (wtA > wtB ? wtA : wtB) : wtC);\n";
-    o << "      const float bm = wave_max(ok ? (m4 > wtD ? m4 : wtD) : ninf);\n";
+    o << "      const float bm = wave_max_ordered(ok ? (m4 > wtD ? m4 : wtD) : ninf);  // (wt starts at +0: never -0)\n";
     o << "      if (max_partials && threadIdx.x == 0) max_partials[row] = bm;\n";
     o << "      if (row_e) {\n";
     o << "        const int32_t eb = row_anchor(bm);\n";
diff --git a/include/gjx.h b/include/gjx.h
--- a/include/gjx.h
+++ b/include/gjx.h
@@ -167,6 +167,7 @@
 int gjx_plan_set_params(gjx_plan* p, const float* params , int n_params);
 #define GJX_SOURCE_FUSED_TAIL 0x100
 #define GJX_SOURCE_WT_STORES 0x200
+#define GJX_SOURCE_FULL_OUTPUTS 0x400
 int gjx_plan_specialized_source(const gjx_plan* p, int impl, char* buf, size_t buf_len, size_t* needed);
 int gjx_plan_prepare(gjx_plan* p, const gjx_keys* particle_keys);
 int gjx_plan_compile_check(const gjx_plan* p, int impl);
```

Measured after the change: 99.48 billion (median of 6 runs). +2.2%, better.
